# blue-yonder/tsfresh

Hardware: AMD Instinct MI355X
Metric: series/sec (ComprehensiveFCParameters, len=1024) (higher is better)
Workload: dtype f64; 1 GPU; 100000 series/GPU x len 1024 float32 i.i.d. N(0,1), ComprehensiveFCParameters (783 columns), inputs and outputs resident in HBM; n_series_per_gpu=100000, length=1024, n_cols=783, parallelism=ids1

## Files before the change

### __graft_entry__.py

```python
import os
import subprocess
import sys

ROOT = os.path.dirname(os.path.abspath(__file__))
if ROOT not in sys.path:
    sys.path.insert(0, ROOT)


def build():
    subprocess.check_call(["make", "-C", os.path.join(ROOT, "tsfresh_amd", "csrc"), "-j4"])
    subprocess.check_call(["make", "-C", os.path.join(ROOT, "tsfresh_amd", "csrc"), "lab"])
    sys.path.insert(0, os.path.join(ROOT, "tests"))
    import emul_lib
    emul_lib.load()
    import emul_pack_lib
    emul_pack_lib.load()
    import emul_pack_set_lib
    emul_pack_set_lib.load()
    import emul_pack_dense_lib
    emul_pack_dense_lib.load()
    import emul_roll_lib
    emul_roll_lib.load()
    import emul_mprofile_lib
    emul_mprofile_lib.load()
    import tsfresh_amd
    from tsfresh_amd import _native
    lib = _native.load()
    for sym in _native.EXPORTS:
        getattr(lib, sym)
    assert lib.tsfa_calc_count() > 70


def smoke():
    import numpy as np
    import pandas as pd

    sys.path.insert(0, os.path.join(ROOT, "tests"))
    from oracle.extract import oracle_matrix
    from parity import compare
    from tsfresh_amd import ComprehensiveFCParameters, _native, extract_features

    if _native.device_count() < 1:
        raise RuntimeError("smoke() needs a HIP device: tsfresh_amd has no CPU fallback")
    rng = np.random.default_rng(7)
    n_ids, length = 16, 256
    x = rng.standard_normal((n_ids, length), dtype=np.float32)
    df = pd.DataFrame({"id": np.repeat(np.arange(n_ids), length), "time": np.tile(np.arange(length), n_ids),
                       "value": x.reshape(-1)})
    params = ComprehensiveFCParameters()
    feats = extract_features(df, column_id="id", column_sort="time", default_fc_parameters=params, device=0)
    assert feats.shape == (n_ids, 783), feats.shape
    values = x.astype(np.float64).reshape(-1)
    offsets = np.arange(n_ids + 1, dtype=np.int64) * length
    names, want = oracle_matrix(values, offsets, params)
    got = feats[names].to_numpy()
    bad = compare(names, got, want, [values[offsets[i]:offsets[i + 1]] for i in range(n_ids)])
    if bad:
        raise AssertionError("%d mismatches vs oracle, e.g. %s" % (len(bad), bad[:5]))
    print("smoke ok: %d series x %d features match the oracle" % feats.shape)


if __name__ == "__main__":
    build()
    if len(sys.argv) > 1 and sys.argv[1] == "smoke":
        smoke()
```

### tsfresh_amd/csrc/fam_ar.h

```cpp
#ifndef TSFA_FAM_AR_H
#define TSFA_FAM_AR_H

#include "tsfa_common.h"

TSFA_DEV int adf_maxlag_for(int n) {
    int maxlag = (int)ceil(12.0 * pow((double)n / 100.0, 0.25));
    const int cap = n / 2 - 1 - 1;
    if (cap < maxlag) maxlag = cap;
    return maxlag;
}

TSFA_DEV int ar_tri(int i, int j) { return ((i * (i + 1)) >> 1) + j; }
TSFA_DEV int ar_tri_doubles(int P) { return (P * (P - 1)) / 2; }

TSFA_DEV void ar_sync(const Blk &b) {
#if TSFA_GPU && !defined(TSFA_LONG)
    if (b.nt <= 64) {
        asm volatile("s_waitcnt lgkmcnt(0)" ::: "memory");
        return;
    }
#endif
    (void)b;
    blk_sync();
}

TSFA_DEV bool chol_factor(double *G, int p) {
    for (int j = 0; j < p; ++j) {
        double d = G[ar_tri(j, j)];
        for (int k = 0; k < j; ++k) d -= G[ar_tri(j, k)] * G[ar_tri(j, k)];
        if (!(d > 0.0)) return false;
        d = sqrt(d);
        G[ar_tri(j, j)] = d;
        for (int i = j + 1; i < p; ++i) {
            double s = G[ar_tri(i, j)];
            for (int k = 0; k < j; ++k) s -= G[ar_tri(i, k)] * G[ar_tri(j, k)];
            G[ar_tri(i, j)] = s / d;
        }
    }
    return true;
}
TSFA_DEV void chol_solve(const double *L, int p, const double *rhs, double *x) {
    for (int i = 0; i < p; ++i) {
        double s = rhs[i];
        for (int k = 0; k < i; ++k) s -= L[ar_tri(i, k)] * x[k];
        x[i] = s * (1.0 / L[ar_tri(i, i)]);
    }
    for (int i = p - 1; i >= 0; --i) {
        double s = x[i];
        for (int k = i + 1; k < p; ++k) s -= L[ar_tri(k, i)] * x[k];
        x[i] = s * (1.0 / L[ar_tri(i, i)]);
    }
}

TSFA_DEV void blk_chol_solve(const Blk &b, const double *L, int p, const double *rhs, double *x) {
#if TSFA_GPU
    const int lane = b.tid & 63;
    const bool live = lane < p;
    double s = live ? rhs[lane] : 0.0;
    const double dg = live ? 1.0 / L[ar_tri(lane, lane)] : 1.0;
    for (int k = 0; k < p; ++k) {
        const double wk = readlane_f64(s, k) * readlane_f64(dg, k);
        if (lane == k) s = wk;
        else if (live && lane > k) s -= L[ar_tri(lane, k)] * wk;
    }
    for (int k = p - 1; k >= 0; --k) {
        const double xk = readlane_f64(s, k) * readlane_f64(dg, k);
        if (lane == k) s = xk;
        else if (live && lane < k) s -= L[ar_tri(k, lane)] * xk;
    }
    if (b.tid < p) x[b.tid] = s;
#else
    if (b.tid == 0) chol_solve(L, p, rhs, x);
#endif
}

#define TSFA_AR_PIVOT_TOL 1e-6
TSFA_DEV bool blk_chol_factor(const Blk &b, double *G, int p, double *diag0, double *dmin = nullptr) {
    for (int a = b.tid; a < p; a += b.nt) diag0[a] = G[ar_tri(a, a)];
    double dm = TSFA_INF;
    for (int j = 0; j < p; ++j) {
        ar_sync(b);
        const double d = G[ar_tri(j, j)];
        if (!(d > TSFA_AR_PIVOT_TOL * diag0[j])) return false;
        dm = fmin(dm, d);
        if (dmin) *dmin = dm;
        const double sd = sqrt(d);
        ar_sync(b);
        const double rsd = 1.0 / sd;
        for (int i = j + b.tid; i < p; i += b.nt) G[ar_tri(i, j)] = (i == j) ? sd : G[ar_tri(i, j)] * rsd;
        ar_sync(b);
        const int rsh = (b.nt >= 32) ? 5 : 0;
        for (int i = j + 1 + (b.tid & ((1 << rsh) - 1)); i < p; i += (1 << rsh)) {
            const double lij = G[ar_tri(i, j)];
            for (int k = j + 1 + (b.tid >> rsh); k <= i; k += (b.nt >> rsh))
                G[ar_tri(i, k)] = G[ar_tri(i, k)] - lij * G[ar_tri(k, j)];
        }
    }
    ar_sync(b);
    return true;
}
TSFA_DEV void blk_chol_forward(const Blk &b, const double *L, int p, double *w) {
#if TSFA_GPU
    if (p <= 64) {
        const int lane = b.tid & 63;
        const bool live = lane < p;
        double s = live ? w[lane] : 0.0;
        const double dg = live ? 1.0 / L[ar_tri(lane, lane)] : 1.0;
// ... 755 lines not shown
```

### tsfresh_amd/csrc/fam_sort.h

```cpp
#ifndef TSFA_FAM_SORT_H
#define TSFA_FAM_SORT_H

#include "tsfa_common.h"
#include "fam_langevin_dd.h"

template <class S>
TSFA_DEV double np_quantile_sorted(S s, int n, double q) {
    const double vi = (double)(n - 1) * q;
    int prev, next;
    double pf = floor(vi);
    if (vi >= (double)(n - 1)) {
        prev = next = n - 1;
        pf = -1.0;
    } else if (vi < 0.0) {
        prev = next = 0;
        pf = 0.0;
    } else {
        prev = (int)pf;
        next = prev + 1;
    }
    const double gamma = vi - pf;
    const double a = s(prev), c = s(next);
    const double diff = c - a;
    double r = a + diff * gamma;
// ... 154 lines not shown
#pragma unroll
    for (int j = 0; j < DD - 1; ++j) {
        int c = 0;
#pragma unroll
        for (int l = j + 1; l < DD; ++l) c += (r[l] < r[j]) ? 1 : 0;
        f /= (DD - j);
        code += c * f;
    }
    return code;
}
template <class AT>
TSFA_DEV int perm_code(const AT *a, int D, int fact) {
    switch (D) {
    case 2: return perm_code_fixed<2>(a, fact);
    case 3: return perm_code_fixed<3>(a, fact);
    case 4: return perm_code_fixed<4>(a, fact);
    case 5: return perm_code_fixed<5>(a, fact);
    case 6: return perm_code_fixed<6>(a, fact);
    case 7: return perm_code_fixed<7>(a, fact);
    default: break;
    }
    int code = 0, f = fact;
    for (int j = 0; j < D - 1; ++j) {
        int c = 0;
        for (int l = j + 1; l < D; ++l) c += ((double)a[l] < (double)a[j]) ? 1 : 0;
        f /= (D - j);
        code += c * f;
    }
    return code;
}

#define TSFA_FRIEDRICH_MAX_R 64
#define TSFA_FRIEDRICH_MAX_M 3

struct FrDefer {
    double *buf;
    int *count;
    int slot_doubles;
    long long sidx;
    int spec;
    int cap;
};

struct FxScale {
    int s1, s2;
};
TSFA_DEV FxScale fx_scale(double amax, int bits) {
    int e2 = 0;
    (void)frexp(amax, &e2);
    FxScale f;
    f.s1 = 60 - bits - e2;
    f.s2 = f.s1 + 59 - bits;
    return f;
}
TSFA_DEV void fx_split(double v, FxScale f, long long &hi, long long &lo) {
    const double h = rint(ldexp(v, f.s1));
    hi = (long long)h;
    lo = (long long)rint(ldexp(v - ldexp(h, -f.s1), f.s2));
}
TSFA_DEV double fx_value(long long hi, long long lo, FxScale f) {
    const long long hh = hi >> 26, hl = hi - hh * 67108864LL, lh = lo >> 26, ll = lo - lh * 67108864LL;
    const double a = ldexp((double)hh, 26 - f.s1), bq = ldexp((double)hl, -f.s1);
    const double c = ldexp((double)lh, 26 - f.s2), d = ldexp((double)ll, -f.s2);
    double s = c + d;
    double e = d - (s - c);
    double s2 = bq + s;
    double bb = s2 - bq;
    double e2 = (bq - (s2 - bb)) + (s - bb);
    double s3 = a + s2;
    bb = s3 - a;
    double e3 = (a - (s3 - bb)) + (s2 - bb);
    return s3 + (e3 + (e2 + e));
}

template <class XS, class S1>
TSFA_DEV bool friedrich_bin_means(const Blk &b, XS xs, int n, S1 srt1, int r, double *fw) {
    const int ns = n - 1;
    if (ns < 1 || r < 1) return false;
    double *edges = fw;
    double *sx = fw + (r + 1);
    double *sy = sx + r;
    double *cnt = sy + r;
    double *lows = cnt + r + 1;
    blk_sync();
    for (int j = b.tid; j <= r; j += b.nt) {
        const double q = np_linspace_at(0.0, 1.0, r + 1, j);
        edges[j] = pd_quantile_sorted(srt1, ns, q);
    }
    long long *isx = (long long *)(void *)sx, *isy = (long long *)(void *)sy, *icnt = (long long *)(void *)cnt,
              *isxl = (long long *)(void *)lows, *isyl = isxl + r;
    for (int j = b.tid; j < r; j += b.nt) { isx[j] = 0; isy[j] = 0; icnt[j] = 0; isxl[j] = 0; isyl[j] = 0; }
    blk_sync();
    double bad = 0.0;
    for (int j = b.tid; j < r; j += b.nt) bad += (edges[j] < edges[j + 1]) ? 0.0 : 1.0;
    bad = blk_sum(b, bad);
    if (bad > 0.0) return false;
    {
        double amax = fmax(fabs(srt1(0)), fabs(srt1(ns - 1)));
        amax = fmax(amax, fabs(xs[n - 1]));
        int bits = 1;
        while ((1 << bits) < n) ++bits;
        const FxScale fx = fx_scale(amax, bits), fy = fx_scale(2.0 * amax, bits);
        for (int i = b.tid; i < ns; i += b.nt) {
            const double x = xs[i];
            int lo = 0, hi = r + 1;
            while (lo < hi) {
                const int mid = (lo + hi) >> 1;
                if (edges[mid] < x) lo = mid + 1; else hi = mid;
            }
            int bin = lo - 1;
            if (x == edges[0]) bin = 0;
            if (bin < 0 || bin >= r) continue;
            const double dlt = xs[i + 1] - xs[i];
            long long xh, xl, yh, yl;
            fx_split(x, fx, xh, xl);
            fx_split(dlt, fy, yh, yl);
#if TSFA_GPU
            atomicAdd((unsigned long long *)&isx[bin], (unsigned long long)xh);
            atomicAdd((unsigned long long *)&isy[bin], (unsigned long long)yh);
            if (xl != 0) atomicAdd((unsigned long long *)&isxl[bin], (unsigned long long)xl);
            if (yl != 0) atomicAdd((unsigned long long *)&isyl[bin], (unsigned long long)yl);
            atomicAdd((unsigned long long *)&icnt[bin], 1ULL);
#else
            isx[bin] += xh; isy[bin] += yh; isxl[bin] += xl; isyl[bin] += yl; icnt[bin] += 1;
#endif
        }
        blk_sync();
        for (int j = b.tid; j < r; j += b.nt) {
            const double vx = fx_value(isx[j], isxl[j], fx), vy = fx_value(isy[j], isyl[j], fy);
            const double vc = (double)icnt[j];
            sx[j] = vx; sy[j] = vy; cnt[j] = vc;
        }
        blk_sync();
    }
    return true;
}

template <class XS, class S1>
TSFA_DEV void friedrich_coeffs(const Blk &b, XS xs, int n, S1 srt1, int m, int r,
                               double *fw, double *coef, const FrDefer &df) {
    for (int k = 0; k <= m; ++k) coef[k] = TSFA_NAN;
    const int ns = n - 1;
    if (ns < 1 || r < 1 || r > TSFA_FRIEDRICH_MAX_R || m < 1 || m > TSFA_FRIEDRICH_MAX_M) return;
    double *sx = fw + (r + 1);
    double *sy = sx + r;
    double *cnt = sy + r;
    double *flag = cnt + r;
    double *A = flag + 1;
    double *yv = A + r * (m + 1);
    double *cc = yv + r;
    double *tmp = cc + (m + 1);
    if (!friedrich_bin_means(b, xs, n, srt1, r, fw)) return;
    if (b.tid == 0) flag[0] = 0.0;
    blk_sync();
    const int rmax = (df.slot_doubles - TSFA_PF_HDR) / 2;
#if TSFA_GPU
    if (b.tid < 64) {
        const int lane = b.tid;
        const bool has = (lane < r) && (cnt[lane < r ? lane : 0] > 0.0);
        const unsigned long long mask = __ballot(has);
        const int k = __popcll(mask);
        const int cols = m + 1;
        const int row = has ? __popcll(mask & ((1ull << lane) - 1ull)) : 1000;
        const double xm = has ? sx[lane] / cnt[lane] : 0.0;
        const double ym = has ? sy[lane] / cnt[lane] : 0.0;
        bool defer = (k < cols);
        if (k >= cols) {
            double yrow = ym;
            double a[TSFA_FRIEDRICH_MAX_M + 1], scale[TSFA_FRIEDRICH_MAX_M + 1], R[TSFA_FRIEDRICH_MAX_M + 1][TSFA_FRIEDRICH_MAX_M + 1],
                qy[TSFA_FRIEDRICH_MAX_M + 1];
#pragma unroll
            for (int c = 0; c <= TSFA_FRIEDRICH_MAX_M; ++c) {
                a[c] = 0.0;
                scale[c] = 1.0;
                if (c < cols) {
                    double pw = 1.0;
                    for (int e = 0; e < m - c; ++e) pw *= xm;
                    pw = has ? pw : 0.0;
                    scale[c] = sqrt(wave_sum(pw * pw));
                    a[c] = pw / scale[c];
                    if (!has) a[c] = 0.0;
                }
            }
            double rmin = TSFA_INF, rbig = 0.0;
#pragma unroll
            for (int kk = 0; kk <= TSFA_FRIEDRICH_MAX_M; ++kk) {
                if (kk < cols) {
                    const bool below = has && (row >= kk);
                    const double nrm = sqrt(wave_sum(below ? a[kk] * a[kk] : 0.0));
                    const double akk = wave_sum((row == kk) ? a[kk] : 0.0);
                    if (nrm != 0.0) {
                        const double alpha = (akk > 0.0) ? -nrm : nrm;
                        const double v0 = akk - alpha;
                        const double vi = (row == kk) ? v0 : ((has && row > kk) ? a[kk] : 0.0);
                        const double vtv = wave_sum(vi * vi);
#pragma unroll
                        for (int j = 0; j <= TSFA_FRIEDRICH_MAX_M; ++j) {
                            if (j > kk && j < cols) {
                                const double d = 2.0 * wave_sum(vi * a[j]) / vtv;
                                a[j] -= d * vi;
                            }
                        }
                        const double d = 2.0 * wave_sum(vi * yrow) / vtv;
                        yrow -= d * vi;
                        R[kk][kk] = alpha;
                    } else {
                        R[kk][kk] = akk;
                    }
                    rmin = fmin(rmin, fabs(R[kk][kk]));
                    rbig = fmax(rbig, fabs(R[kk][kk]));
#pragma unroll
                    for (int j = 0; j <= TSFA_FRIEDRICH_MAX_M; ++j)
                        if (j > kk && j < cols) R[kk][j] = wave_sum((row == kk) ? a[j] : 0.0);
                    qy[kk] = wave_sum((row == kk) ? yrow : 0.0);
                }
            }
            double sol[TSFA_FRIEDRICH_MAX_M + 1];
#pragma unroll
            for (int kk = TSFA_FRIEDRICH_MAX_M; kk >= 0; --kk) {
                sol[kk] = 0.0;
                if (kk < cols) {
                    double sacc = qy[kk];
#pragma unroll
                    for (int j = 0; j <= TSFA_FRIEDRICH_MAX_M; ++j)
                        if (j > kk && j < cols) sacc -= R[kk][j] * sol[j];
                    sol[kk] = sacc / R[kk][kk];
                }
            }
            if (lane == 0) {
#pragma unroll
                for (int c = 0; c <= TSFA_FRIEDRICH_MAX_M; ++c)
                    if (c < cols) cc[c] = sol[c] / scale[c];
                flag[0] = 1.0;
            }
            defer = (rmin < TSFA_PF_FLAG * rbig);
        }
        if (defer && k >= 1) {
            if (df.buf != nullptr && r <= rmax) {
                int slot = 0;
                if (lane == 0) slot = atomicAdd(df.count, 1);
                slot = __shfl(slot, 0);
                if (slot < df.cap) {
                    double *rec = df.buf + (size_t)slot * (size_t)df.slot_doubles;
                    if (lane == 0) { rec[0] = (double)df.sidx; rec[1] = (double)df.spec; rec[2] = (double)k; }
                    if (has) { rec[TSFA_PF_HDR + row] = xm; rec[TSFA_PF_HDR + rmax + row] = ym; }
                }
            }
        }
    }
#else
    if (b.tid == 0) {
        int k = 0;
        double ysave[TSFA_FRIEDRICH_MAX_R];
        for (int j = 0; j < r; ++j) {
            if (cnt[j] > 0.0) {
                tmp[k] = sx[j] / cnt[j];
                yv[k] = sy[j] / cnt[j];
                ysave[k] = yv[k];
                ++k;
            }
        }
        const int cols = m + 1;
        double scale[TSFA_FRIEDRICH_MAX_M + 1];
        for (int c = 0; c < cols; ++c) {
            double ss = 0.0;
            for (int i = 0; i < k; ++i) {
                double pw = 1.0;
                for (int e = 0; e < m - c; ++e) pw *= tmp[i];
                A[i + c * k] = pw;
                ss += pw * pw;
            }
            scale[c] = sqrt(ss);
            for (int i = 0; i < k; ++i) A[i + c * k] /= scale[c];
        }
        bool defer = (k < cols);
        if (k >= cols) {
            double xsave[TSFA_FRIEDRICH_MAX_R];
            for (int i = 0; i < k; ++i) xsave[i] = tmp[i];
            small_lstsq(A, k, cols, yv, cc, tmp);
            for (int c = 0; c < cols; ++c) cc[c] = cc[c] / scale[c];
            flag[0] = 1.0;
            double rmin = TSFA_INF, rbig = 0.0;
            for (int c = 0; c < cols; ++c) {
                rmin = fmin(rmin, fabs(A[c + c * k]));
                rbig = fmax(rbig, fabs(A[c + c * k]));
            }
            defer = (rmin < TSFA_PF_FLAG * rbig);
            for (int i = 0; i < k; ++i) tmp[i] = xsave[i];
        }
        if (defer && k >= 1) {
            (void)rmax;
            double cf[TSFA_PF_MAXC];
            const double *tx = tmp;
            polyfit_svd_dd([=](int i) { return tx[i]; }, [=](int i) { return ysave[i]; }, k, m, cf);
            for (int c = 0; c < cols; ++c) cc[c] = cf[c];
            flag[0] = 1.0;
        }
    }
#endif
    blk_sync();
    if (flag[0] != 0.0)
        for (int c = 0; c <= m; ++c) coef[c] = cc[c];
    blk_sync();
}

#define TSFA_CQ_REFINE 9.5367431640625e-07
#ifdef TSFA_EMUL
static long long g_tsfa_cq_refined = 0;
#define TSFA_CQ_REFINE_NOTE() (++g_tsfa_cq_refined)
#else
#define TSFA_CQ_REFINE_NOTE() ((void)0)
#endif
struct CqRefined { double v, va; };
template <class XS>
TSFA_DEVN CqRefined cq_refine_corridor(const Blk &b, XS xs, int n, double l, double h, double mu1, double mu2, double c) {
    double e[4] = {0.0, 0.0, 0.0, 0.0};
    for (int i = b.tid; i < n - 1; i += b.nt) {
        const double x0 = xs[i], x1 = xs[i + 1];
        if (x0 >= l && x0 <= h && x1 >= l && x1 <= h) {
            const double d = x1 - x0;
            const double e1 = d - mu1, e2 = fabs(d) - mu2;
            e[0] += e1;
            e[1] += e1 * e1;
            e[2] += e2;
            e[3] += e2 * e2;
        }
    }
    blk_sum_multi<4>(b, e);
    CqRefined r;
    r.v = (e[1] - e[0] * e[0] / c) / c;
    r.va = (e[3] - e[2] * e[2] / c) / c;
    return r;
}
template <class XS, class SS>
TSFA_DEV void cq_fill_all(const Blk &b, XS xs, SS srt, int n, const TsfaCqPlan &plan, double *cq) {
    TSFA_TICKER(tkq, 0);
    for (int e0 = 0; e0 < 2 * plan.n; e0 += b.nt) {
        const int e = e0 + b.tid;
        double q = 0.0;
#if TSFA_GPU
        for (int c = 0; c < plan.n; ++c) {
            q = (e == c) ? plan.ql[c] : q;
            q = (e == plan.n + c) ? plan.qh[c] : q;
        }
#else
        if (e < 2 * plan.n) q = (e < plan.n) ? plan.ql[e] : plan.qh[e - plan.n];
#endif
        if (e < 2 * plan.n) {
            const double v = pd_quantile_sorted([=](int i) { return srt[i]; }, n, q);
            if (e < plan.n) cq[5 * e] = v; else cq[5 * (e - plan.n) + 1] = v;
        }
    }
    blk_sync();
    double s = (n > 1) ? (xs[n - 1] - xs[0]) / (double)(n - 1) : 0.0;
    if (!(fabs(s) <= 1.7976931348623157e308)) s = 0.0;
    const double sa = fabs(s);
    TSFA_TICK(tkq, b, 220);
    for (int k0 = 0; k0 < plan.n; k0 += 4) {
        const int ng = (plan.n - k0 < 4) ? (plan.n - k0) : 4;
        double lo[4], hi[4];
#pragma unroll
        for (int j = 0; j < 4; ++j) {
            const int k = (j < ng) ? (k0 + j) : k0;
            double l = cq[5 * k], h = cq[5 * k + 1];
#if TSFA_GPU
            l = readlane_f64(l, 0);
            h = readlane_f64(h, 0);
#endif
            lo[j] = (j < ng) ? l : TSFA_INF;
            hi[j] = (j < ng) ? h : -TSFA_INF;
        }
        double a[20];
#pragma unroll
        for (int k = 0; k < 20; ++k) a[k] = 0.0;
        for (int i = b.tid; i < n - 1; i += b.nt) {
            const double x0 = xs[i], x1 = xs[i + 1];
            const double d = x1 - x0;
            const double dd = d - s, ad = fabs(d) - sa;
            const double dd2 = dd * dd, ad2 = ad * ad;
#pragma unroll
            for (int j = 0; j < 4; ++j) {
                if (x0 >= lo[j] && x0 <= hi[j] && x1 >= lo[j] && x1 <= hi[j]) {
                    a[5 * j] += 1.0;
                    a[5 * j + 1] += dd;
                    a[5 * j + 2] += ad;
                    a[5 * j + 3] += dd2;
                    a[5 * j + 4] += ad2;
                }
            }
        }
        TSFA_TICK(tkq, b, 221);
        blk_sum_multi<20>(b, a);
        TSFA_TICK(tkq, b, 222);
        int refine = 0;
#pragma unroll
        for (int j = 0; j < 4; ++j) {
            const double c = a[5 * j], q1 = a[5 * j + 3] * c, q2 = a[5 * j + 4] * c;
            const bool many = c > 1.0;
            refine |= (many && q1 - a[5 * j + 1] * a[5 * j + 1] < TSFA_CQ_REFINE * q1) ? (1 << j) : 0;
            refine |= (many && q2 - a[5 * j + 2] * a[5 * j + 2] < TSFA_CQ_REFINE * q2) ? (16 << j) : 0;
        }
#if TSFA_GPU
        refine = __builtin_amdgcn_readfirstlane(refine);
#endif
        for (int j = 0; refine != 0 && j < ng; ++j) {
            if (((refine >> j) & 0x11) == 0) continue;
            TSFA_CQ_REFINE_NOTE();
            double l = lo[0], h = hi[0], c = a[0], t1 = a[1], t2 = a[2];
#pragma unroll
            for (int jj = 1; jj < 4; ++jj) {
                l = (jj == j) ? lo[jj] : l;
                h = (jj == j) ? hi[jj] : h;
                c = (jj == j) ? a[5 * jj] : c;
                t1 = (jj == j) ? a[5 * jj + 1] : t1;
                t2 = (jj == j) ? a[5 * jj + 2] : t2;
            }
            const CqRefined w = cq_refine_corridor(b, xs, n, l, h, s + t1 / c, sa + t2 / c, c);
            const double w1 = w.v, w2 = w.va;
#pragma unroll
            for (int jj = 0; jj < 4; ++jj) {
                a[5 * jj + 3] = (jj == j && ((refine >> jj) & 1)) ? w1 : a[5 * jj + 3];
                a[5 * jj + 4] = (jj == j && ((refine >> jj) & 16)) ? w2 : a[5 * jj + 4];
            }
        }
        blk_sync();
        if (b.tid == 0) {
#pragma unroll
            for (int j = 0; j < 4; ++j) {
                if (j < ng) {
                    double *o = cq + 5 * (k0 + j);
                    const double c = a[5 * j];
                    const bool any = c > 0.0;
                    const double m1 = any ? a[5 * j + 1] / c : 0.0, m2 = any ? a[5 * j + 2] / c : 0.0;
                    o[0] = c;
                    o[1] = any ? s + m1 : 0.0;
                    o[2] = any ? sa + m2 : 0.0;
                    double v1 = a[5 * j + 3] / c - m1 * m1, v2 = a[5 * j + 4] / c - m2 * m2;
                    v1 = ((refine >> j) & 1) ? a[5 * j + 3] : v1;
                    v2 = ((refine >> j) & 16) ? a[5 * j + 4] : v2;
                    o[3] = any ? ((v1 < 0.0) ? 0.0 : v1) : 0.0;
                    o[4] = any ? ((v2 < 0.0) ? 0.0 : v2) : 0.0;
                }
            }
        }
    }
    blk_sync();
}

enum { TSFA_SCTX_SYM = 0, TSFA_SCTX_NUNIQUE, TSFA_SCTX_MULTI_VALS, TSFA_SCTX_MULTI_PTS, TSFA_SCTX_SUM_VALS, TSFA_SCTX_SUM_PTS,
       TSFA_SORT_CTX = 8 };

template <class SS>
TSFA_DEV void sort_epilogue(const Blk &b, const TsfaSpec *specs, int first, int nspecs, int n, SS srt, const double *ctx,
                            const double *cq, double *out_row) {
    const double dn = (double)n;
    const double vmin = srt[0], vmax = srt[n - 1];
    for (int s = first + b.tid; s < nspecs; s += b.nt) {
        const TsfaSpec sp = specs[s];
        const double p0 = sp.p[0];
        double v = TSFA_NAN;
        switch (sp.calc) {
        case TSFA_C_MEDIAN: v = (n & 1) ? srt[(n - 1) / 2] : (0.0 + srt[n / 2 - 1] + srt[n / 2]) / 2.0; break;
        case TSFA_C_QUANTILE: v = np_quantile_sorted([=](int i) { return srt[i]; }, n, p0); break;
        case TSFA_C_SYMMETRY_LOOKING: v = (ctx[TSFA_SCTX_SYM] < p0 * (vmax - vmin)) ? 1.0 : 0.0; break;
        case TSFA_C_CHANGE_QUANTILES: {
            if (sp.p[1] != -2.0) { v = 0.0; break; }
            const double *o = cq + 5 * (((int)p0) & 127);
            const bool isabs = (sp.p[2] != 0.0);
            if (o[0] == 0.0) v = 0.0;
            else if ((int)sp.p[3] == TSFA_AGG_MEAN) v = isabs ? o[2] : o[1];
            else v = isabs ? o[4] : o[3];
        } break;
        case TSFA_C_HAS_DUPLICATE: v = (ctx[TSFA_SCTX_NUNIQUE] != dn) ? 1.0 : 0.0; break;
        case TSFA_C_RATIO_VALUE_NUMBER: v = ctx[TSFA_SCTX_NUNIQUE] / dn; break;
        case TSFA_C_PCT_REOCC_VALUES: v = ctx[TSFA_SCTX_MULTI_VALS] / ctx[TSFA_SCTX_NUNIQUE]; break;
        case TSFA_C_PCT_REOCC_DATAPOINTS: v = ctx[TSFA_SCTX_MULTI_PTS] / dn; break;
        case TSFA_C_SUM_REOCC_VALUES: v = ctx[TSFA_SCTX_SUM_VALS]; break;
        case TSFA_C_SUM_REOCC_DATA_POINTS: v = ctx[TSFA_SCTX_SUM_PTS]; break;
        default: break;
        }
        out_row[sp.col] = v;
    }
}

template <class ST>
TSFA_DEV void fam_sort_series(const Blk &b, const ST *xs_raw, int n, const TsfaSpec *specs, int nspecs,
                              double *out_row, ST *srt_raw, double *w, int *iw, const TsfaCqPlan &cqplan, double *cq,
                              TsfaSpec *stage, int n_loop = -1, double *ctx = nullptr, int w_doubles = 1280,
                              FrDefer df = FrDefer{nullptr, nullptr, TSFA_PF_HDR + 2 * TSFA_FRIEDRICH_MAX_R, 0, 0},
                              const unsigned short *perm_in = nullptr, const double *stats = nullptr, int pe_hint = 0) {
    const int hist_words = 2 * w_doubles;
    const int nloop = (n_loop >= 0 && ctx != nullptr) ? n_loop : nspecs;
    const XsView<ST> xs{xs_raw};
    const XsView<ST> srt{srt_raw};
    const int np2 = next_pow2(n);
    TSFA_TICKER(tk, 0);
    blk_sync();
    auto build_sorted_copy = [&]() {
        if (perm_in != nullptr && n >= 3) {
            for (int i = b.tid; i < np2; i += b.nt) srt_raw[i] = (i < n) ? xs_raw[perm_in[i]] : (ST)TSFA_INF;
            blk_sync();
        } else
#if TSFA_GPU
        if (!blk_sorted_copy_regs(b, xs_raw, n, srt_raw, np2))
#endif
        {
            for (int i = b.tid; i < np2; i += b.nt) srt_raw[i] = (i < n) ? xs_raw[i] : (ST)TSFA_INF;
            blk_bitonic_sort(b, srt_raw, np2);
        }
    };
    build_sorted_copy();
    TSFA_TICK(tk, b, 104);
    const double dn = (double)n;
    const double vmin = srt[0], vmax = srt[n - 1];

    bool have_sym = false, cq_valid = false, fr_valid = false;
    double sym_dist = 0.0, cq_ql = 0.0, cq_qh = 0.0, cq_cnt = 0.0, cq_mean = 0.0, cq_mean_abs = 0.0, cq_var = 0.0, cq_var_abs = 0.0;
    int fr_m = 0, fr_r = 0;
    double fr_coef[TSFA_FRIEDRICH_MAX_M + 1];

    double n_unique = 0.0, n_multi_vals = 0.0, n_multi_pts = 0.0, sum_multi_vals = 0.0, sum_multi_pts = 0.0;
    bool have_runs = false;

    for (int s = 0; s < nloop; ++s) {
        const TsfaSpec sp = spec_fetch(b, specs, nspecs, s, stage);
        const double p0 = sp.p[0], p1 = sp.p[1], p2 = sp.p[2], p3 = sp.p[3];
        double v = TSFA_NAN;
        switch (sp.calc) {
        case TSFA_C_MEDIAN:
            v = (n & 1) ? srt[(n - 1) / 2] : (0.0 + srt[n / 2 - 1] + srt[n / 2]) / 2.0;
            break;
        case TSFA_C_QUANTILE:
            v = np_quantile_sorted([=](int i) { return srt[i]; }, n, p0);
            break;
        case TSFA_C_SYMMETRY_LOOKING: {
            if (!have_sym) {
                const double mean = stats ? stats[TSFA_STATS_MEAN] : np_sum(b, n, [=](int i) { return xs[i]; }) / dn;
                const double med = (n & 1) ? srt[(n - 1) / 2] : (0.0 + srt[n / 2 - 1] + srt[n / 2]) / 2.0;
                sym_dist = fabs(mean - med);
                have_sym = true;
                if (nloop < nspecs && b.tid == 0) ctx[TSFA_SCTX_SYM] = sym_dist;
            }
            v = (sym_dist < p0 * (vmax - vmin)) ? 1.0 : 0.0;
        } break;
        case TSFA_C_MEAN_N_ABSOLUTE_MAX: {
            const int k = (int)p0;
            double r = TSFA_NAN;
            if (b.tid == 0 && n > k) {
                int lo = 0, hi = n - 1;
                double acc = 0.0;
                for (int t = 0; t < k; ++t) {
                    const double a = fabs(srt[lo]), c = fabs(srt[hi]);
                    if (a > c) { acc += a; ++lo; } else { acc += c; --hi; }
                }
                r = acc / (double)k;
            }
            v = blk_bcast0(b, r);
        } break;
        case TSFA_C_CHANGE_QUANTILES: {
            const double ql = p0, qh = p1;
            const bool isabs = (p2 != 0.0);
            const int agg = (int)p3;
            if (cqplan.n > 0 && p1 == -2.0) {
                if ((int)p0 >= 128) cq_fill_all(b, xs, srt, n, cqplan, cq);
                const double *o = cq + 5 * (((int)p0) & 127);
                if (o[0] == 0.0) v = 0.0;
                else if (agg == TSFA_AGG_MEAN) v = isabs ? o[2] : o[1];
                else v = isabs ? o[4] : o[3];
                break;
            }
            if (ql >= qh) { v = 0.0; break; }
            if (!(cq_valid && cq_ql == ql && cq_qh == qh)) {
                const double lo = pd_quantile_sorted([=](int i) { return srt[i]; }, n, ql);
                const double hi = pd_quantile_sorted([=](int i) { return srt[i]; }, n, qh);
                double c = 0.0, a = 0.0, aa = 0.0;
                for (int i = b.tid; i < n - 1; i += b.nt) {
                    const double x0 = xs[i], x1 = xs[i + 1];
                    if (x0 >= lo && x0 <= hi && x1 >= lo && x1 <= hi) {
                        const double d = x1 - x0;
                        c += 1.0;
                        a += d;
                        aa += fabs(d);
                    }
                }
                c = blk_sum(b, c);
                a = blk_sum(b, a);
                aa = blk_sum(b, aa);
                cq_cnt = c;
                cq_mean = (c > 0.0) ? a / c : 0.0;
                cq_mean_abs = (c > 0.0) ? aa / c : 0.0;
                double ss = 0.0, ssa = 0.0;
                if (c > 0.0) {
                    const double m1 = cq_mean, m2 = cq_mean_abs;
                    for (int i = b.tid; i < n - 1; i += b.nt) {
                        const double x0 = xs[i], x1 = xs[i + 1];
                        if (x0 >= lo && x0 <= hi && x1 >= lo && x1 <= hi) {
                            const double d = x1 - x0;
                            ss += (d - m1) * (d - m1);
                            ssa += (fabs(d) - m2) * (fabs(d) - m2);
                        }
                    }
                    ss = blk_sum(b, ss);
                    ssa = blk_sum(b, ssa);
                }
                cq_var = (c > 0.0) ? ss / c : 0.0;
                cq_var_abs = (c > 0.0) ? ssa / c : 0.0;
                cq_valid = true;
                cq_ql = ql;
                cq_qh = qh;
            }
            if (cq_cnt == 0.0) v = 0.0;
            else if (agg == TSFA_AGG_MEAN) v = isabs ? cq_mean_abs : cq_mean;
            else v = isabs ? cq_var_abs : cq_var;
        } break;
        case TSFA_C_HAS_DUPLICATE:
        case TSFA_C_RATIO_VALUE_NUMBER:
        case TSFA_C_PCT_REOCC_VALUES:
        case TSFA_C_PCT_REOCC_DATAPOINTS:
        case TSFA_C_SUM_REOCC_VALUES:
        case TSFA_C_SUM_REOCC_DATA_POINTS: {
            if (!have_runs) {
                double nu = 0.0, mv = 0.0, mp = 0.0, sv = 0.0, spn = 0.0;
                for (int i = b.tid; i < n; i += b.nt) {
                    const double x = srt[i];
                    const bool eq_prev = (i > 0) && (srt[i - 1] == x);
                    const bool eq_next = (i < n - 1) && (srt[i + 1] == x);
                    if (!eq_prev) {
                        nu += 1.0;
                        if (eq_next) { mv += 1.0; sv += x; }
                    }
                    if (eq_prev || eq_next) { mp += 1.0; spn += x; }
                }
                double r5[5] = {nu, mv, mp, sv, spn};
                blk_sum_multi<5>(b, r5);
                n_unique = r5[0]; n_multi_vals = r5[1]; n_multi_pts = r5[2]; sum_multi_vals = r5[3]; sum_multi_pts = r5[4];
                have_runs = true;
                if (nloop < nspecs && b.tid == 0) {
                    ctx[TSFA_SCTX_NUNIQUE] = n_unique; ctx[TSFA_SCTX_MULTI_VALS] = n_multi_vals;
                    ctx[TSFA_SCTX_MULTI_PTS] = n_multi_pts; ctx[TSFA_SCTX_SUM_VALS] = sum_multi_vals;
                    ctx[TSFA_SCTX_SUM_PTS] = sum_multi_pts;
                }
            }
            if (sp.calc == TSFA_C_HAS_DUPLICATE) v = (n_unique != dn) ? 1.0 : 0.0;
            else if (sp.calc == TSFA_C_RATIO_VALUE_NUMBER) v = n_unique / dn;
            else if (sp.calc == TSFA_C_PCT_REOCC_VALUES) v = n_multi_vals / n_unique;
            else if (sp.calc == TSFA_C_PCT_REOCC_DATAPOINTS) v = n_multi_pts / dn;
            else if (sp.calc == TSFA_C_SUM_REOCC_VALUES) v = sum_multi_vals;
            else v = sum_multi_pts;
        } break;
        case TSFA_C_PERMUTATION_ENTROPY: {
            const int tau = (int)p0, D = (int)p1;
            if (pe_hint != 0) { TSFA_TICK(tk, b, sp.calc); continue; }
            const int num = (n >= D) ? ((n - D) / tau + 1) : 0;
            if (num <= 0) { v = TSFA_NAN; break; }
            int fact = 1;
            for (int k = 2; k <= D; ++k) fact *= k;
            const bool wide = num > 65535;
            const int per_pass = wide ? hist_words : 2 * hist_words;
            if (fact > 16 * per_pass && sizeof(ST) >= sizeof(int)) {
                int *codes_s = (int *)(void *)srt_raw;
                const int cp2 = next_pow2(num);
                blk_sync();
                for (int t = b.tid; t < cp2; t += b.nt) codes_s[t] = (t < num) ? perm_code(xs_raw + t * tau, D, fact) : 0x7FFFFFFF;
                blk_bitonic_sort(b, codes_s, cp2);
                double es = 0.0;
                for (int t = b.tid; t < num; t += b.nt) {
                    const int c0 = codes_s[t];
                    if (t > 0 && codes_s[t - 1] == c0) continue;
                    int lo = t + 1, hi = num;
                    while (lo < hi) { const int mid = (lo + hi) >> 1; if (codes_s[mid] > c0) hi = mid; else lo = mid + 1; }
                    const double pr = (double)(lo - t) / (double)num;
                    es += pr * log(pr);
                }
                v = -blk_sum(b, es);
                blk_sync();
                build_sorted_copy();
                break;
            }
            const bool in_regs = (num <= 8 * b.nt);
            TSFA_TICKER(tp, 0);
            int codes[8];
            if (in_regs) {
#pragma unroll
                for (int u = 0; u < 8; ++u) {
                    const int t = b.tid + u * b.nt;
                    codes[u] = (t < num) ? perm_code(xs_raw + t * tau, D, fact) : -1;
                }
            }
            TSFA_TICK(tp, b, 236);
            const int LT = 64;
            double *ltab = b.np->leaf_sum;
            blk_sync();
            for (int c = b.tid; c < LT; c += b.nt) ltab[c] = (c > 0) ? log((double)c / (double)num) : 0.0;
            blk_sync();
            TSFA_TICK(tp, b, 237);
            double e = 0.0;
            for (int base = 0; base < fact; base += per_pass) {
                const int top = (fact - base < per_pass) ? (fact - base) : per_pass;
                blk_sync();
                for (int k = b.tid; k < (wide ? top : (top + 1) >> 1); k += b.nt) iw[k] = 0;
                blk_sync();
                if (in_regs) {
#pragma unroll
                    for (int u = 0; u < 8; ++u) {
                        const int c = codes[u] - base;
                        if (codes[u] >= 0 && c >= 0 && c < top) {
#if TSFA_GPU
                            if (wide) atomicAdd(&iw[c], 1); else atomicAdd(&iw[c >> 1], (c & 1) ? 0x10000 : 1);
#else
                            if (wide) iw[c] += 1; else iw[c >> 1] += (c & 1) ? 0x10000 : 1;
#endif
                        }
                    }
                } else {
                    for (int t = b.tid; t < num; t += b.nt) {
                        const int c = perm_code(xs_raw + t * tau, D, fact) - base;
                        if (c >= 0 && c < top) {
#if TSFA_GPU
                            if (wide) atomicAdd(&iw[c], 1); else atomicAdd(&iw[c >> 1], (c & 1) ? 0x10000 : 1);
#else
                            if (wide) iw[c] += 1; else iw[c >> 1] += (c & 1) ? 0x10000 : 1;
#endif
                        }
                    }
                }
                blk_sync();
                if (fact <= num) {
                    for (int k = b.tid; k < top; k += b.nt) {
                        const unsigned wv = (unsigned)iw[wide ? k : (k >> 1)];
                        const int c = wide ? (int)wv : ((k & 1) ? (int)(wv >> 16) : (int)(wv & 0xffffu));
                        if (c > 0) {
                            const double pr = (double)c / (double)num;
                            e += pr * ((c < LT) ? ltab[c] : log(pr));
                        }
                    }
                } else {
                    double acc = 0.0;
                    if (in_regs) {
#pragma unroll
                        for (int u = 0; u < 8; ++u) {
                            const int c = codes[u] - base;
                            if (codes[u] >= 0 && c >= 0 && c < top) {
                                const unsigned wv = (unsigned)iw[wide ? c : (c >> 1)];
                                const int cc = wide ? (int)wv : ((c & 1) ? (int)(wv >> 16) : (int)(wv & 0xffffu));
                                acc += (cc < LT) ? ltab[cc] : log((double)cc / (double)num);
                            }
                        }
                    } else {
                        for (int t = b.tid; t < num; t += b.nt) {
                            const int c = perm_code(xs_raw + t * tau, D, fact) - base;
                            if (c >= 0 && c < top) {
                                const unsigned wv = (unsigned)iw[wide ? c : (c >> 1)];
                                const int cc = wide ? (int)wv : ((c & 1) ? (int)(wv >> 16) : (int)(wv & 0xffffu));
                                acc += (cc < LT) ? ltab[cc] : log((double)cc / (double)num);
                            }
                        }
                    }
                    e += acc / (double)num;
                }
            }
            TSFA_TICK(tp, b, 238);
            v = -blk_sum(b, e);
            TSFA_TICK(tp, b, 239);
        } break;
        case TSFA_C_FRIEDRICH_COEFFICIENTS:
        case TSFA_C_MAX_LANGEVIN_FIXED_POINT: {
            int coeff, m, r;
            if (sp.calc == TSFA_C_FRIEDRICH_COEFFICIENTS) { coeff = (int)p0; m = (int)p1; r = (int)p2; }
            else { coeff = -1; m = (int)p0; r = (int)p1; }
            if (!(fr_valid && fr_m == m && fr_r == r)) {
                int pos = 0;
                {
                    const double xl = xs[n - 1];
                    int lo = 0, hi = n;
                    while (lo < hi) {
                        const int mid = (lo + hi) >> 1;
                        if (srt[mid] < xl) lo = mid + 1; else hi = mid;
                    }
                    pos = lo;
                }
                const XsView<ST> sr = srt;
                df.spec = s;
                friedrich_coeffs(b, xs, n, [=](int i) { return sr[i < pos ? i : i + 1]; }, m, r, w, fr_coef, df);
                fr_valid = true;
                fr_m = m;
                fr_r = r;
            }
            const double *coef = fr_coef;
            if (sp.calc == TSFA_C_FRIEDRICH_COEFFICIENTS) v = (coeff >= 0 && coeff <= m && m <= TSFA_FRIEDRICH_MAX_M) ? coef[coeff] : TSFA_NAN;
            else v = (m >= 1 && m <= TSFA_FRIEDRICH_MAX_M) ? max_real_root_deg3(coef, m + 1) : TSFA_NAN;
        } break;
        default: break;
        }
        if (b.tid == 0) out_row[sp.col] = v;
        TSFA_TICK(tk, b, sp.calc);
    }
    if (nloop < nspecs) {
        blk_sync();
        sort_epilogue(b, specs, nloop, nspecs, n, srt, ctx, cq, out_row);
    }
}

#endif
```

### tsfresh_amd/csrc/tsfa_api.cpp

```cpp
#include <hip/hip_runtime.h>

#include <stdio.h>
#include <stdlib.h>

#include <algorithm>
#include <string>
#include <vector>

#include "../../include/tsfresh_amd.h"
#include "tsfa_host_tables.h"
#include "tsfa_launch.h"
#include "fam_seq.h"
#include "tsfa_layout.h"

static thread_local std::string g_last_error;

static int fail(int code, const std::string &msg) {
    g_last_error = msg;
    return code;
}

int tsfa_fail(int code, const char *msg) { return fail(code, std::string(msg ? msg : "")); }
#define HIP_TRY(expr)                                                                                    \
    do {                                                                                                 \
        hipError_t e_ = (expr);                                                                          \
        if (e_ != hipSuccess) return fail(TSFA_ERR_HIP, std::string(#expr) + ": " + hipGetErrorString(e_)); \
    } while (0)

struct DevBuf {
    void *p = nullptr;
    size_t cap = 0;
    int ensure(size_t bytes) {
        if (bytes <= cap) return 0;
        size_t want = bytes + bytes / 8 + 4096;
        void *q = nullptr;
        if (hipMalloc(&q, want) != hipSuccess) {
            (void)hipGetLastError();
            if (p) { (void)hipFree(p); p = nullptr; cap = 0; }
            if (hipMalloc(&q, want) != hipSuccess) {
                (void)hipGetLastError();
                return -1;
            }
        }
        if (p) (void)hipFree(p);
        p = q;
        cap = want;
        return 0;
    }
    void release() {
        if (p) (void)hipFree(p);
        p = nullptr;
        cap = 0;
    }
};

#define TSFA_MAX_AUX 3
#define TSFA_MAX_CHUNKS 16
#define TSFA_DEFAULT_STREAMS 1

struct Timing {
    std::string name;
    hipEvent_t e0 = nullptr, e1 = nullptr;
    float ms = 0.f;
};

struct PlanOptions {
    bool length_classes = true;
    bool stats_share = true;
    bool perm_share = true;
    bool select = true;
    bool bluestein = true;
    bool cwt_mfma = false;
    bool force_long = false;
    int entropy_route = 0;
    int bluestein_min = 0;
    int gscratch_slots = 0;
    int host_chunks = 0;
    int nt[TSFA_N_FAMILIES] = {0};
    bool trace = false;
    bool row_form = true;
    int seq_rows = -1;
};

#if defined(TSFA_LAB)
#define TSFA_LAB_ONLY(x) (x)
#else
#define TSFA_LAB_ONLY(x) (0)
#endif

static int64_t g_relevance_batch = 0;
int64_t tsfa_relevance_batch_override() { return g_relevance_batch; }

struct tsfa_plan {
    int device = 0;
    PlanOptions opt;
    hipStream_t stream = nullptr;
    int n_cols = 0;
    std::vector<TsfaSpec> fam_specs[TSFA_N_FAMILIES];
    TsfaSpec *d_specs[TSFA_N_FAMILIES] = {nullptr};
    TsfaFamHints hints[TSFA_N_FAMILIES];
    TsfaCwtBank bank;
    double *d_W = nullptr;
    int *d_cols = nullptr, *d_coeff = nullptr;
    double *d_dectab = nullptr, *d_twc = nullptr, *d_tws = nullptr, *d_consts = nullptr;
    long long *d_stats = nullptr;
    DevBuf values, offsets, out, gscratch, times, deg_list, sel, long_scratch, pf_buf, perm_buf, stats_buf, dd_scratch, gen_scratch, seq_rows;
    std::vector<TsfaSpec> gen_specs;
    TsfaSpec *d_gen_specs = nullptr;
    TsfaGenPlan gen_plan;
    double *d_pool = nullptr;
    int *d_deg_count = nullptr;
    int *d_cursor = nullptr;
    hipStream_t s_in = nullptr, s_out = nullptr;
    hipEvent_t ev_in[TSFA_MAX_CHUNKS] = {nullptr}, ev_k[TSFA_MAX_CHUNKS] = {nullptr};
    std::vector<int64_t> h_rel;
    bool needs_times = false;
    bool sort_only_order_stats = false;
    bool stream_ok = false;
    int n_streams = 1;
    hipStream_t aux[TSFA_MAX_AUX] = {nullptr};
    hipEvent_t ev_fork = nullptr, ev_join[TSFA_MAX_AUX] = {nullptr};
    bool profiling = false;
    std::vector<Timing> timings;
    std::vector<tsfa_launch_info> launches;
    long long hint_min_len = 0, hint_max_len = 0;
    bool fill_all = false;
    int *d_fill_cols = nullptr;
    int n_fill_cols = 0;
    int debug_skip_fam = -1;
    hipStream_t side = nullptr;
    hipEvent_t ev_side_fork = nullptr, ev_side_join = nullptr;
    unsigned side_mask = 0;
    double fill_value = __builtin_nan("");
};

static const char *fam_names[TSFA_N_FAMILIES] = {"k_basic", "k_sort", "k_spectral", "k_ar", "k_entropy", "k_cwtpeaks", "k_seq", "k_trend", "k_mprofile"};

template <class T>
static int upload(const std::vector<T> &h, T **d) {
    *d = nullptr;
    if (h.empty()) return 0;
    if (hipMalloc((void **)d, h.size() * sizeof(T)) != hipSuccess) return -1;
    if (hipMemcpy(*d, h.data(), h.size() * sizeof(T), hipMemcpyHostToDevice) != hipSuccess) return -1;
    return 0;
}

static int record(tsfa_plan *plan, hipStream_t st, size_t slot, const char *name, bool begin) {
    if (!plan->profiling) return 0;
    if (plan->timings.size() <= slot) plan->timings.resize(slot + 1);
    Timing &t = plan->timings[slot];
    if (!t.e0) {
        if (hipEventCreate(&t.e0) != hipSuccess || hipEventCreate(&t.e1) != hipSuccess) return -1;
// ... 157 lines not shown
    for (int f = 0; ok && f < TSFA_N_FAMILIES; ++f) ok = upload(plan->fam_specs[f], &plan->d_specs[f]) == 0;
    if (ok) ok = upload(plan->gen_specs, &plan->d_gen_specs) == 0;
    if (ok && n_data > 0) ok = upload(std::vector<double>(data, data + n_data), &plan->d_pool) == 0;
    if (ok && !cwt_coef.empty()) {
        ok = upload(plan->bank.W, &plan->d_W) == 0 && upload(plan->bank.cols, &plan->d_cols) == 0 &&
             upload(plan->bank.coeff_idx, &plan->d_coeff) == 0;
    }
    if (ok) {
        std::vector<double> dt, twc, tws;
        tsfa_build_dectab(dt);
        tsfa_build_twiddles(twc, tws);
        ok = upload(dt, &plan->d_dectab) == 0 && upload(twc, &plan->d_twc) == 0 && upload(tws, &plan->d_tws) == 0;
        std::vector<double> consts;
        tsfa_build_consts(consts);
        ok = ok && upload(consts, &plan->d_consts) == 0;
    }
    if (ok) ok = hipMalloc((void **)&plan->d_stats, TSFA_LEN_STATS * sizeof(long long)) == hipSuccess;
    if (ok) ok = hipMalloc((void **)&plan->d_deg_count, 2 * sizeof(int)) == hipSuccess;
    if (ok) ok = hipMalloc((void **)&plan->d_cursor, TSFA_N_LEN_CLASSES * sizeof(int)) == hipSuccess;
    if (ok) ok = hipStreamCreateWithFlags(&plan->s_in, hipStreamNonBlocking) == hipSuccess &&
                 hipStreamCreateWithFlags(&plan->s_out, hipStreamNonBlocking) == hipSuccess;
    for (int i = 0; ok && i < TSFA_MAX_CHUNKS; ++i)
        ok = hipEventCreateWithFlags(&plan->ev_in[i], hipEventDisableTiming) == hipSuccess &&
             hipEventCreateWithFlags(&plan->ev_k[i], hipEventDisableTiming) == hipSuccess;
    {
        const char *e = getenv("TSFA_STREAMS");
        plan->n_streams = e ? std::min(std::max(atoi(e), 1), TSFA_MAX_AUX + 1) : TSFA_DEFAULT_STREAMS;
        for (int i = 0; ok && i + 1 < plan->n_streams; ++i)
            ok = hipStreamCreateWithFlags(&plan->aux[i], hipStreamNonBlocking) == hipSuccess &&
                 hipEventCreateWithFlags(&plan->ev_join[i], hipEventDisableTiming) == hipSuccess;
        if (ok && plan->n_streams > 1) ok = hipEventCreateWithFlags(&plan->ev_fork, hipEventDisableTiming) == hipSuccess;
    }
    if (const char *e = getenv("TSFA_PAIR")) {
        static const char *nm[TSFA_N_FAMILIES] = {"basic", "sort", "spectral", "ar", "entropy", "cwt", "seq", "trend", "mprofile"};
        for (int f = 0; f < TSFA_N_FAMILIES; ++f)
            if (f != TSFA_FAM_BASIC && f != TSFA_FAM_SORT && f != TSFA_FAM_ENTROPY && strstr(e, nm[f])) plan->side_mask |= 1u << f;
        if (plan->side_mask) {
            int least = 0, greatest = 0;
            (void)hipDeviceGetStreamPriorityRange(&least, &greatest);
            ok = ok && hipStreamCreateWithPriority(&plan->side, hipStreamNonBlocking, least) == hipSuccess &&
                 hipEventCreateWithFlags(&plan->ev_side_fork, hipEventDisableTiming) == hipSuccess &&
                 hipEventCreateWithFlags(&plan->ev_side_join, hipEventDisableTiming) == hipSuccess;
        }
    }
    if (const char *e = getenv("TSFA_HOST_CHUNKS")) plan->opt.host_chunks = std::max(atoi(e), 0);
    if (!ok) {
        tsfa_plan_destroy(plan);
        return fail(TSFA_ERR_HIP, "device allocation/upload failed while creating the plan");
    }
    *out_plan = plan;
    return TSFA_OK;
}

int32_t tsfa_plan_n_cols(const tsfa_plan *plan) { return plan ? plan->n_cols : -1; }

int tsfa_plan_set_length_hint(tsfa_plan *plan, int64_t min_len, int64_t max_len) {
    if (!plan) return fail(TSFA_ERR_INVALID, "null plan");
    if (max_len == 0 && min_len == 0) { plan->hint_min_len = plan->hint_max_len = 0; return TSFA_OK; }
    if (min_len < 1 || max_len < min_len || max_len > 2147483647LL / 64) return fail(TSFA_ERR_INVALID, "length hint must satisfy 1 <= min <= max <= 33554431");
    plan->hint_min_len = min_len;
    plan->hint_max_len = max_len;
    return TSFA_OK;
}

int tsfa_plan_set_option(tsfa_plan *plan, const char *name, double value) {
    if (!name) return fail(TSFA_ERR_INVALID, "option name is NULL");
    const std::string n(name);
    const bool on = value != 0.0;
    if (!plan) {
        if (n == "relevance_batch") { g_relevance_batch = value > 0.0 ? (int64_t)value : 0; return TSFA_OK; }
        return fail(TSFA_ERR_INVALID, "unknown library option '" + n + "'");
    }
    PlanOptions &o = plan->opt;
    if (n == "length_classes") o.length_classes = on;
    else if (n == "stats_share") o.stats_share = on;
    else if (n == "perm_share") o.perm_share = on;
    else if (n == "select") o.select = on;
    else if (n == "bluestein") o.bluestein = on;
    else if (n == "cwt_mfma") o.cwt_mfma = on;
    else if (n == "force_long") o.force_long = on;
    else if (n == "row_form") o.row_form = on;
    else if (n == "seq_rows") o.seq_rows = (value < 0.0) ? -1 : (on ? 1 : 0);
    else if (n == "entropy_route") { if (value != 0.0 && value != 1.0 && value != 2.0) return fail(TSFA_ERR_INVALID, "entropy_route: 0, 1 or 2"); o.entropy_route = (int)value; }
    else if (n == "bluestein_min") o.bluestein_min = value > 0.0 ? (int)std::min(value, 32767.0) : 0;
    else if (n == "gscratch_slots") o.gscratch_slots = value > 0.0 ? (int)std::min(value, 2147483647.0) : 0;
    else if (n == "host_chunks") o.host_chunks = value > 0.0 ? (int)std::min(value, (double)TSFA_MAX_CHUNKS) : 0;
    else if (n == "fused_minimal") { if (!on) plan->stream_ok = false; }
    else if (n == "perm_fused") { if (!on) plan->hints[TSFA_FAM_SORT].d = 0; }
    else if (n == "fill") { plan->fill_value = value; plan->fill_all = true; }
    else if (n == "fill_off") { plan->fill_all = false; }
#if defined(TSFA_LAB)
    else if (n == "skip_family") plan->debug_skip_fam = (int)value;
    else if (n == "trace") o.trace = on;
    else if (n.rfind("nt_", 0) == 0 && n.size() == 4 && n[3] >= '0' && n[3] < '0' + TSFA_N_FAMILIES) o.nt[n[3] - '0'] = (int)value;
#endif
    else return fail(TSFA_ERR_INVALID, "unknown plan option '" + n + "'");
    return TSFA_OK;
}

int tsfa_plan_set_profiling(tsfa_plan *plan, int32_t enable) {
    if (!plan) return fail(TSFA_ERR_INVALID, "plan is NULL");
    plan->profiling = enable != 0;
    return TSFA_OK;
}

int32_t tsfa_plan_last_timings(const tsfa_plan *plan, const char **names, float *ms, int32_t cap) {
    if (!plan) return 0;
    int32_t n = 0;
    for (const auto &t : plan->timings) {
        if (n >= cap) break;
        if (names) names[n] = t.name.c_str();
        if (ms) ms[n] = t.ms;
        ++n;
    }
    return n;
}

int32_t tsfa_plan_last_launches(const tsfa_plan *plan, tsfa_launch_info *out, int32_t cap) {
    if (!plan) return 0;
    const int32_t n = (int32_t)plan->launches.size();
    for (int32_t i = 0; out && i < n && i < cap; ++i) out[i] = plan->launches[(size_t)i];
    return n;
}

int tsfa_extract(tsfa_plan *plan, const void *values, int32_t dtype, const int64_t *offsets, int64_t n_series,
                 double *out, int64_t ld_out, int32_t space, void *stream) {
    return tsfa_extract_timed(plan, values, dtype, nullptr, offsets, n_series, out, ld_out, space, stream);
}

int tsfa_extract_timed(tsfa_plan *plan, const void *values, int32_t dtype, const double *times, const int64_t *offsets,
                       int64_t n_series, double *out, int64_t ld_out, int32_t space, void *stream) {
    return tsfa_extract_windows(plan, values, dtype, times, offsets, offsets ? offsets + 1 : nullptr, n_series, out,
                                ld_out, space, stream);
}

struct BatchShape {
    long long max_len = 0, min_len = 0, max_np2 = 0;
    int n_groups = 1;
    int g_maxn[TSFA_N_LEN_CLASSES] = {0};
    long long g_np2[TSFA_N_LEN_CLASSES] = {0};
    int64_t g_count[TSFA_N_LEN_CLASSES] = {0};
    bool g_has_short[TSFA_N_LEN_CLASSES] = {false};
    TsfaClassMap map;
};

static void shape_from_stats(const long long *st, int64_t n_series, BatchShape &sh, bool length_classes) {
    sh.max_len = st[0];
    sh.min_len = st[1];
    sh.max_np2 = st[2];
    memset(&sh.map, 0, sizeof sh.map);
    sh.n_groups = 1;
    sh.g_maxn[0] = (int)st[0];
    sh.g_np2[0] = st[2];
    sh.g_count[0] = n_series;
    sh.g_has_short[0] = st[1] <= TSFA_ROW_MAXN;
    if (!length_classes || n_series < 2048 || st[0] <= 2 * st[1] || st[0] <= 128) return;
    const int64_t min_group = 512;
    int ng = 0;
    int64_t pend_count = 0;
    long long pend_np2 = 0;
    int first_of_group = 0;
    for (int c = 0; c < TSFA_N_LEN_CLASSES; ++c) {
        const int64_t cnt = st[3 + c];
        pend_count += cnt;
        pend_np2 = std::max(pend_np2, st[3 + 2 * TSFA_N_LEN_CLASSES + c]);
        bool last = true;
// ... 61 lines not shown

static int run_batch(tsfa_plan *plan, const void *d_values, int dtype, const double *d_times, const int64_t *d_starts,
                     const int64_t *d_ends, int64_t n_series, double *d_out, int64_t ld, const BatchShape &sh,
                     const int *d_sel, hipStream_t st, bool with_overlap) {
    if ((plan->fill_all || plan->n_fill_cols > 0) &&
        tsfa_launch_fill_nan(d_out, n_series, plan->n_cols, ld, st, plan->fill_value, plan->fill_all ? nullptr : plan->d_fill_cols,
                             plan->n_fill_cols))
        return fail(TSFA_ERR_HIP, "fill launch failed");

    static const int order_long_first[TSFA_N_FAMILIES] = {TSFA_FAM_ENTROPY, TSFA_FAM_AR, TSFA_FAM_SORT, TSFA_FAM_CWT, TSFA_FAM_BASIC,
                                                          TSFA_FAM_SEQ, TSFA_FAM_SPECTRAL, TSFA_FAM_TREND, TSFA_FAM_MPROFILE};
    static const int order_basic_first[TSFA_N_FAMILIES] = {TSFA_FAM_BASIC, TSFA_FAM_ENTROPY, TSFA_FAM_AR, TSFA_FAM_SORT, TSFA_FAM_CWT,
                                                           TSFA_FAM_SEQ, TSFA_FAM_SPECTRAL, TSFA_FAM_TREND, TSFA_FAM_MPROFILE};
    const bool overlap = with_overlap && plan->n_streams > 1 && !plan->profiling;
    const bool share_stats = plan->stats_buf.p != nullptr && !overlap && !plan->stream_ok && plan->opt.stats_share;
    const int *order = share_stats ? order_basic_first : order_long_first;
    bool stats_valid[TSFA_N_LEN_CLASSES + 1];
    for (int g = 0; g <= TSFA_N_LEN_CLASSES; ++g) stats_valid[g] = false;
    if (overlap) {
        HIP_TRY(hipEventRecord(plan->ev_fork, st));
        for (int i = 0; i + 1 < plan->n_streams; ++i) HIP_TRY(hipStreamWaitEvent(plan->aux[i], plan->ev_fork, 0));
    }
    bool pair = plan->side != nullptr && plan->side_mask != 0 && !overlap && !plan->profiling && with_overlap;
    for (int g = 0; g < sh.n_groups; ++g) pair = pair && sh.g_maxn[g] <= 4096;
    bool side_forked = false, side_used = false;
    size_t slot = 0;
    int dealt = 0;
    bool perm_valid[TSFA_N_LEN_CLASSES + 1];
    for (int g = 0; g <= TSFA_N_LEN_CLASSES; ++g) perm_valid[g] = false;
    const bool perm_share = plan->perm_buf.p != nullptr && !overlap && plan->opt.perm_share;
    bool stream_done[TSFA_N_LEN_CLASSES + 1];
    for (int g = 0; g <= TSFA_N_LEN_CLASSES; ++g) stream_done[g] = false;
    for (int fi = 0; fi < TSFA_N_FAMILIES; ++fi) {
        const int f = order[fi];
        if (plan->fam_specs[f].empty()) continue;
        if (TSFA_LAB_ONLY(plan->debug_skip_fam == f)) continue;
        if (f == TSFA_FAM_BASIC && plan->stream_ok) {
            bool all = true;
            for (int g = 0; g < sh.n_groups; ++g) all = all && stream_done[g];
            if (all) continue;
        }
        hipStream_t fst = st;
        if (overlap) {
            const int k = dealt++ % plan->n_streams;
            if (k > 0) fst = plan->aux[k - 1];
        }
        if (pair && fi > 0 && ((plan->side_mask >> f) & 1u)) {
            if (!side_forked) {
                HIP_TRY(hipEventRecord(plan->ev_side_fork, st));
                HIP_TRY(hipStreamWaitEvent(plan->side, plan->ev_side_fork, 0));
                side_forked = true;
            }
            fst = plan->side;
            side_used = true;
        }
        const char *slot_name = (plan->stream_ok && (f == TSFA_FAM_SORT || (f == TSFA_FAM_BASIC && plan->fam_specs[TSFA_FAM_SORT].empty())))
                                    ? "k_stream" : fam_names[f];
        if (record(plan, fst, slot, slot_name, true)) return fail(TSFA_ERR_HIP, "event record failed");
        std::vector<TsfaLaunch> perm_launches;
        for (int g = sh.n_groups - 1; g >= 0; --g) {
            const int maxn = sh.g_maxn[g];
            const long long max_np2 = sh.g_np2[g];
            TsfaLaunch a;
            memset(&a, 0, sizeof a);
            a.fam = f;
            a.dtype = dtype;
            a.values = d_values;
            a.starts = d_starts;
            a.ends = d_ends;
            a.n_series = sh.g_count[g];
            a.sel = (sh.n_groups > 1) ? d_sel + sh.map.base[g] : nullptr;
            a.specs = plan->d_specs[f];
            a.nspecs = (int)plan->fam_specs[f].size();
            a.out = d_out;
            a.ld = ld;
            a.maxn = maxn;
            a.nt = (maxn <= 2048) ? 64 : 256;
            if (maxn > 2048) {
                static const int nt_8k[TSFA_N_FAMILIES] = {512, 512, 512, 512, 256, 1024, 256, 256, 256};
                static const int nt_4k[TSFA_N_FAMILIES] = {256, 256, 256, 256, 256, 512, 256, 256, 256};
                a.nt = (maxn > 4096) ? nt_8k[f] : nt_4k[f];
            }
            if (maxn <= 2048) {
                static const int pref[TSFA_N_FAMILIES] = {64, 128, 128, 64, 256, 256, 128, 64, 256};
                const int cap = std::max(64, ((maxn / 4 + 63) / 64) * 64);
                a.nt = std::min(pref[f], cap);
            }
            if (TSFA_LAB_ONLY(plan->opt.nt[f] >= 64)) a.nt = plan->opt.nt[f];
            a.stream = fst;
            a.dectab = plan->d_dectab;
            a.times = d_times;
            a.twc = plan->d_twc;
            a.consts = plan->d_consts;
            a.tws = plan->d_tws;
            a.hint_a = plan->hints[f].a;
            a.hint_b = plan->hints[f].b;
            a.hint_c = plan->hints[f].c;
            a.hint_d = plan->hints[f].d;
            a.hint_e = plan->hints[f].e;
            a.alt = plan->hints[f].alt;
            a.cq = plan->hints[f].cq;
            if (f == TSFA_FAM_SPECTRAL && maxn > 2048 && !TSFA_LAB_ONLY(plan->opt.nt[f] >= 64)) a.nt = 512;
            int aux = 0;
            if (f == TSFA_FAM_TREND) aux = a.alt.small_w;
            if (f == TSFA_FAM_MPROFILE) aux = (dtype == TSFA_F32) ? 4 : 8;
            if (f == TSFA_FAM_SPECTRAL) {
                a.dft_n = (int)std::min<long long>(max_np2, 256);
                aux = a.dft_n;
                int bl_odd = TSFA_BLUESTEIN_MIN, bl_even = TSFA_BLUESTEIN_MIN_EVEN;
                if (plan->opt.bluestein_min > 0) bl_odd = bl_even = std::min(std::max(plan->opt.bluestein_min, 17), 32767);
                a.bluestein_min = TSFA_BLUESTEIN_PACK(bl_odd, bl_even);
                if (max_np2 >= std::min(bl_odd, bl_even) && max_np2 <= 32768 && plan->opt.bluestein) {
                    long long M = 1;
                    while (M < 2 * max_np2 - 1) M <<= 1;
                    const size_t slot_bytes = (size_t)(4 * M) * sizeof(double);
                    int64_t slots = std::min<int64_t>(a.n_series, std::max<int64_t>((int64_t)((1ull << 30) / slot_bytes), 2048));
                    if (plan->opt.gscratch_slots > 0) slots = std::min<int64_t>(slots, plan->opt.gscratch_slots);
                    const size_t bytes = (size_t)slots * slot_bytes;
                    if (plan->gscratch.ensure(bytes) == 0) {
                        a.gscratch = (double *)plan->gscratch.p;
                        a.gscratch_n = (int)(4 * M);
                        a.gscratch_slots = slots;
                    }
                }
            } else if (f == TSFA_FAM_CWT) {
                a.cwt_rowv = tsfa_family_lds_bytes(f, maxn, a.nt, 1) <= 96 * 1024 ? 1 : 0;
                aux = a.cwt_rowv;
                if (plan->opt.cwt_mfma) a.cwt_rowv |= 2;
            } else if (f == TSFA_FAM_AR) {
                int P = 8, Pdd = 8;
                for (const auto &s : plan->fam_specs[f]) {
                    if (s.calc == TSFA_C_AUGMENTED_DICKEY_FULLER) {
                        int ml = (int)ceil(12.0 * pow((double)maxn / 100.0, 0.25));
                        if (maxn / 2 - 2 < ml) ml = maxn / 2 - 2;
                        P = std::max(P, ml + 3);
                    } else if (s.calc == TSFA_C_AR_COEFFICIENT) {
                        const int k = std::min((int)s.p[1], std::max(1, (maxn - 2) / 2));
                        if ((int)s.p[1] <= TSFA_AR_TABLE_K) P = std::max(P, (int)s.p[1] + 2);
                        Pdd = std::max(Pdd, k + 2);
                        a.ar_has_coef = 1;
                    }
                }
                Pdd = std::max(Pdd, P);
                a.ar_P = P;
                a.ar_P_dd = Pdd;
                aux = P;
                {
                    ArDdLds D;
                    if (D.carve(nullptr, Pdd) > TSFA_LDS_LIMIT - 2048) {
                        const size_t slot_bytes = (size_t)ArDdLds::scratch_doubles(Pdd) * sizeof(double);
                        const int slots = (int)std::min<int64_t>(a.n_series, std::min<int64_t>(256, std::max<int64_t>(8, (int64_t)(((size_t)2 << 30) / slot_bytes))));
                        if (plan->dd_scratch.ensure((size_t)slots * slot_bytes))
                            return fail(TSFA_ERR_HIP, "hipMalloc failed for the second AR pass");
                        a.dd_scratch = (double *)plan->dd_scratch.p;
                        a.dd_slots = slots;
                    }
                }
                a.deg_list = (long long *)plan->deg_list.p;
                a.deg_count = plan->d_deg_count;
                HIP_TRY(hipMemsetAsync(plan->d_deg_count, 0, sizeof(int), fst));
            } else if (f == TSFA_FAM_SORT && plan->hints[f].b > 0) {
                a.pf_slot = tsfa_pf_slot_doubles(plan->hints[f].b);
                a.pf_buf = (double *)plan->pf_buf.p;
                a.pf_count = plan->d_deg_count + 1;
                a.pf_cap = (int)std::min<long long>((long long)n_series * std::max(1, plan->hints[f].e), 2147483647LL);
                HIP_TRY(hipMemsetAsync(a.pf_count, 0, sizeof(int), fst));
            } else if (f == TSFA_FAM_ENTROPY) {
                const int waves = std::min(4, std::max(1, (maxn - 1 + 63) / 64));
                a.nt = std::max(a.nt, 64 * waves);
// ... 52 lines not shown
                    for (int s0 = 0; s0 < a.nspecs; s0 += group_g) {
                        lz_build_group(plan->fam_specs[f].data() + s0, std::min(group_g, a.nspecs - s0), maxn, &g, 1);
                        lds_g = std::max(lds_g, tsfa_seq_lds_bytes(g));
                        stride_g = std::max(stride_g, (size_t)g.stride);
                    }
                    auto resident = [&](size_t lds) {
                        if (lds > TSFA_LDS_LIMIT) return (size_t)0;
                        return std::min<size_t>((size_t)(163840 / std::max<size_t>(lds, 1)), (size_t)(32 * 64 / a.nt));
                    };
                    const bool more = resident(lds_g) > resident(seq_lds);
                    if (lds_g <= TSFA_LDS_LIMIT && (plan->opt.seq_rows == 1 || more) &&
                        (size_t)a.n_series * stride_g <= ((size_t)2 << 30) &&
                        plan->seq_rows.ensure((size_t)a.n_series * stride_g) == 0) {
                        seq_grows = 1;
                        seq_group = group_g;
                        seq_lds = lds_g;
                        a.seq_rows = (unsigned char *)plan->seq_rows.p;
                    }
                }
            }
            size_t lds = (f == TSFA_FAM_SEQ) ? seq_lds
                         : (f == TSFA_FAM_ENTROPY) ? tsfa_entropy_lds_bytes(maxn, a.ent_cnt)
                                                   : tsfa_family_lds_bytes(f, maxn, a.nt, aux);
            const bool use_long = lds > TSFA_LDS_LIMIT || plan->opt.force_long || (f == TSFA_FAM_ENTROPY && a.ent_cnt == 4);
            if (TSFA_LAB_ONLY(f == TSFA_FAM_SPECTRAL && plan->opt.trace))
                fprintf(stderr, "[tsfa] spectral group %d: n_series %lld maxn %d max_np2 %lld lds %zu long %d chirp-z %d slots %lld nt %d\n", g,
                        (long long)a.n_series, maxn, max_np2, lds, (int)use_long, (int)(a.gscratch != nullptr), (long long)a.gscratch_slots, a.nt);
            if (use_long) {
                if (!(f == TSFA_FAM_ENTROPY && a.ent_cnt == 4)) a.nt = 256;
                if (a.gscratch != nullptr && a.gscratch_slots < std::min<int64_t>(a.n_series, 2048)) a.gscratch = nullptr;
                if (f == TSFA_FAM_ENTROPY && a.ent_cnt != 4) { a.ent_cnt = 0; a.ent_fast = 0; lds = tsfa_entropy_lds_bytes(maxn, 5); }
                if (f == TSFA_FAM_CWT) { a.cwt_rowv &= 2; lds = tsfa_family_lds_bytes(f, maxn, a.nt, 0); }
                if (f == TSFA_FAM_SEQ) {
                    seq_group = std::min(a.nspecs, TSFA_LZ_MAX_GROUP);
                    seq_grows = 0;
                    lds = 0;
                    for (int s0 = 0; s0 < a.nspecs; s0 += seq_group) {
                        lz_build_group(plan->fam_specs[f].data() + s0, std::min(seq_group, a.nspecs - s0), maxn, &a.seq);
                        lds = std::max(lds, tsfa_seq_lds_bytes(a.seq));
                    }
                } else if (f != TSFA_FAM_ENTROPY && f != TSFA_FAM_CWT) {
                    lds = tsfa_family_lds_bytes(f, maxn, a.nt, aux);
                }
                const size_t slot_bytes = (lds + 255) & ~(size_t)255;
                const int64_t n_slots = std::max<int64_t>(1, std::min<int64_t>(std::min<int64_t>(a.n_series, 512),
                                                                               (int64_t)((4ull << 30) / slot_bytes)));
                if (plan->long_scratch.ensure((size_t)n_slots * slot_bytes))
                    return fail(TSFA_ERR_HIP, "hipMalloc failed for the long-series scratch");
                a.long_scratch = (unsigned char *)plan->long_scratch.p;
                a.long_bytes = (size_t)n_slots * slot_bytes;
            }
            if (share_stats && g <= TSFA_N_LEN_CLASSES) {
                if (f == TSFA_FAM_BASIC && !(plan->hints[f].c == 0 && a.nt <= 256)) {
                    a.stats_out = (double *)plan->stats_buf.p;
                    stats_valid[g] = true;
                } else if ((f == TSFA_FAM_ENTROPY || f == TSFA_FAM_AR || f == TSFA_FAM_SEQ || f == TSFA_FAM_SORT) && stats_valid[g]) {
                    a.stats_in = (const double *)plan->stats_buf.p;
                }
            }
            if (perm_share && !use_long && g <= TSFA_N_LEN_CLASSES) {
                if (f == TSFA_FAM_ENTROPY && a.ent_cnt == 2 && maxn <= TSFA_ENTB_MAXN) {
                    a.perm_buf = (unsigned short *)plan->perm_buf.p;
                    a.perm_stride = TSFA_ENTB_MAXN;
                    perm_valid[g] = true;
                } else if (f == TSFA_FAM_SORT && perm_valid[g]) {
                    a.perm_buf = (unsigned short *)plan->perm_buf.p;
                    a.perm_stride = TSFA_ENTB_MAXN;
                }
            }
            if (f == TSFA_FAM_SORT) {
                a.hint_d = 0;
                if (plan->hints[f].d != 0) {
                    const int pnt = (maxn <= 2048) ? std::min(256, std::max(64, ((maxn / 4 + 63) / 64) * 64))
                                                   : std::min(1024, ((maxn / 8 + 63) / 64) * 64);
                    if (maxn <= 65535 && tsfa_perm_lds_bytes(maxn, pnt, dtype == TSFA_F32 ? 4 : 8) <= TSFA_LDS_LIMIT) {
                        a.hint_d = plan->hints[f].d;
                        TsfaLaunch pa = a;
                        pa.nt = pnt;
                        pa.long_scratch = nullptr;
                        perm_launches.push_back(pa);
                    }
                }
            }
            if (!(plan->stream_ok && (f == TSFA_FAM_SORT || f == TSFA_FAM_BASIC) && maxn <= 2048 && g <= TSFA_N_LEN_CLASSES && stream_done[g])) {
                tsfa_launch_info li;
                li.family = f;
                li.length_class = g;
                li.max_len = maxn;
                li.threads = a.nt;
                li.n_series = a.n_series;
                li.lds_bytes = (int64_t)lds;
                li.long_build = use_long ? 1 : 0;
                li.variant = (f == TSFA_FAM_ENTROPY) ? a.ent_cnt
                             : (f == TSFA_FAM_CWT) ? a.cwt_rowv
                             : (f == TSFA_FAM_SEQ) ? (seq_group | (seq_grows << 8))
                             : (f == TSFA_FAM_SPECTRAL) ? (a.gscratch != nullptr ? 1 : 0)
                             : (f == TSFA_FAM_SORT) ? (a.hint_d != 0 ? 1 : 0)
                             : (f == TSFA_FAM_AR) ? (a.dd_scratch != nullptr ? 1 : 0) : 0;
                plan->launches.push_back(li);
            }
            int rc = 0;
            if (plan->stream_ok && (f == TSFA_FAM_SORT || f == TSFA_FAM_BASIC) && maxn <= 2048 && g <= TSFA_N_LEN_CLASSES) {
                if (stream_done[g]) continue;
                TsfaLaunch sa = a;
                sa.specs = plan->d_specs[TSFA_FAM_SORT];
                sa.nspecs = (int)plan->fam_specs[TSFA_FAM_SORT].size();
                sa.bspecs = plan->d_specs[TSFA_FAM_BASIC];
                sa.nbspecs = (int)plan->fam_specs[TSFA_FAM_BASIC].size();
                rc = tsfa_launch_stream(sa);
                stream_done[g] = true;
            } else
            if (f == TSFA_FAM_SORT && plan->sort_only_order_stats && maxn <= 2048 && !use_long &&
                plan->opt.select) {
                rc = tsfa_launch_order_stats(a);
            } else if (f == TSFA_FAM_SEQ) {
                for (int s0 = 0; rc == 0 && s0 < a.nspecs; s0 += seq_group) {
                    lz_build_group(plan->fam_specs[f].data() + s0, std::min(seq_group, a.nspecs - s0), maxn, &a.seq, seq_grows);
                    if (!use_long && tsfa_seq_lds_bytes(a.seq) > TSFA_LDS_LIMIT)
                        return fail(TSFA_ERR_TOO_LONG, "k_seq: a series of " + std::to_string(maxn) + " samples does not fit LDS");
                    rc = use_long ? tsfa_launch_family_long(a) : tsfa_launch_family(a);
                }
            } else {
                bool rows_any = false, rows_all = false;
                const bool lite = (f == TSFA_FAM_BASIC && plan->hints[f].c == 0 && a.nt <= 256);
                if ((f == TSFA_FAM_BASIC || f == TSFA_FAM_TREND) && plan->opt.row_form && !lite && g <= TSFA_N_LEN_CLASSES) {
                    rows_any = sh.g_has_short[g];
                    rows_all = maxn <= TSFA_ROW_MAXN;
                }
                if (rows_any) {
                    a.skip_le = TSFA_ROW_MAXN;
                    rc = tsfa_launch_rows(a);
                }
                if (rc == 0 && !rows_all) rc = use_long ? tsfa_launch_family_long(a) : tsfa_launch_family(a);
            }
            if (rc == 0 && f == TSFA_FAM_AR) rc = tsfa_launch_ar_degenerate(a);
            if (rc == 0 && f == TSFA_FAM_SORT && a.pf_buf) rc = tsfa_launch_langevin_dd(a);
            if (rc) return fail(TSFA_ERR_HIP, std::string(fam_names[f]) + " launch failed: " +
                                                  (rc == -2 ? "no scratch slot" : hipGetErrorString((hipError_t)rc)));
        }
        if (record(plan, fst, slot, slot_name, false)) return fail(TSFA_ERR_HIP, "event record failed");
        ++slot;
        if (!perm_launches.empty()) {
            if (record(plan, fst, slot, "k_perm", true)) return fail(TSFA_ERR_HIP, "event record failed");
            for (const auto &pa : perm_launches) {
                const int rc = tsfa_launch_perm(pa);
                if (rc) return fail(TSFA_ERR_HIP, std::string("k_perm launch failed: ") + hipGetErrorString((hipError_t)rc));
            }
            if (record(plan, fst, slot, "k_perm", false)) return fail(TSFA_ERR_HIP, "event record failed");
            ++slot;
        }
    }
    if (overlap) {
        for (int i = 0; i + 1 < plan->n_streams; ++i) {
            HIP_TRY(hipEventRecord(plan->ev_join[i], plan->aux[i]));
            HIP_TRY(hipStreamWaitEvent(st, plan->ev_join[i], 0));
        }
    }
    if (side_used) {
        HIP_TRY(hipEventRecord(plan->ev_side_join, plan->side));
        HIP_TRY(hipStreamWaitEvent(st, plan->ev_side_join, 0));
    }
    if (plan->bank.C > 0) {
        TsfaCwtLaunch c;
        memset(&c, 0, sizeof c);
        c.dtype = dtype;
        c.values = d_values;
        c.starts = d_starts;
        c.ends = d_ends;
        c.n_series = n_series;
        c.W = plan->d_W;
        c.S4 = plan->bank.S4;
        c.C = plan->bank.C;
        c.cols = plan->d_cols;
        c.coeff_idx = plan->d_coeff;
        c.out = d_out;
        c.ld = ld;
        c.stream = st;
        if (record(plan, st, slot, "k_cwt_gemm", true)) return fail(TSFA_ERR_HIP, "event record failed");
        const int rc = tsfa_launch_cwt(c);
        if (rc) return fail(TSFA_ERR_HIP, "k_cwt_gemm launch failed");
// ... 237 lines not shown
```

### tsfresh_amd/csrc/tsfa_common.h

```cpp
#ifndef TSFA_COMMON_H
#define TSFA_COMMON_H

#include <math.h>
#include <stdint.h>

#include "tsfa_specs.h"

#if defined(__HIPCC__)
#include <hip/hip_runtime.h>
#define TSFA_GPU 1
#define TSFA_DEV __device__ __forceinline__
#define TSFA_DEVN __device__ __noinline__
#define TSFA_MEM __device__ __forceinline__
#else
#define TSFA_GPU 0
#define TSFA_DEV static inline
#define TSFA_DEVN static
#define TSFA_MEM inline
#endif
#if defined(__HIP_DEVICE_COMPILE__)
#define TSFA_ASSUME_LDS(p) __builtin_assume(__builtin_amdgcn_is_shared((const void *)(p)))
#else
#define TSFA_ASSUME_LDS(p) ((void)0)
#endif
// ... 7 lines not shown
struct NpScratch {
    double leaf_sum[TSFA_NP_MAXLEAF];
    double vst[32];
    int leaf_off[TSFA_NP_MAXLEAF];
    int leaf_len[TSFA_NP_MAXLEAF];
    int st_o[32], st_l[32], st_v[32];
    int nleaf;
    int pad;
    double result;
};

template <typename ST>
struct XsView {
    typedef ST elem;
    const ST *p;
    TSFA_MEM double operator[](int i) const { return (double)p[i]; }
};

struct Blk {
    int tid;
    int nt;
    double *red;
    NpScratch *np;
};

#define TSFA_ROW_MAXN 256
#define TSFA_ROW_LANES 16
struct BlkRow : Blk {};
template <class BT> struct BlkLanes { static constexpr int n = 64; };
template <> struct BlkLanes<BlkRow> { static constexpr int n = TSFA_ROW_LANES; };
template <class BT> struct BlkIsRow { static constexpr bool v = false; };
template <> struct BlkIsRow<BlkRow> { static constexpr bool v = true; };
TSFA_DEV Blk blk_rebind(const Blk &b, int tid) { return Blk{tid, b.nt, b.red, b.np}; }
TSFA_DEV BlkRow blk_rebind(const BlkRow &b, int tid) { BlkRow r; r.tid = tid; r.nt = b.nt; r.red = b.red; r.np = b.np; return r; }

#if TSFA_GPU && defined(TSFA_TICKS)
static __device__ unsigned long long tsfa_ticks[256];
static __shared__ unsigned long long tsfa_ticks_lds[256];
struct Ticker {
    unsigned long long t;
    int base;
    __device__ __forceinline__ explicit Ticker(int base_) : t(__builtin_readcyclecounter()), base(base_) {}
    __device__ __forceinline__ void mark(int tid, int id) {
        const unsigned long long now = __builtin_readcyclecounter();
        if (tid == 0) tsfa_ticks_lds[base + id] += now - t;
        t = __builtin_readcyclecounter();
    }
};
#define TSFA_TICKER(name, base) Ticker name(base)
#define TSFA_TICK(name, b, id) name.mark((b).tid, id)
#define TSFA_TICKS_BEGIN()                                                                  \
    do {                                                                                    \
        for (int i_ = threadIdx.x; i_ < 256; i_ += blockDim.x) tsfa_ticks_lds[i_] = 0ull;   \
        __syncthreads();                                                                    \
    } while (0)
#define TSFA_TICKS_END()                                                                    \
    do {                                                                                    \
        __syncthreads();                                                                    \
        for (int i_ = threadIdx.x; i_ < 256; i_ += blockDim.x)                              \
            if (tsfa_ticks_lds[i_]) atomicAdd(&tsfa_ticks[i_], tsfa_ticks_lds[i_]);         \
    } while (0)
#else
#define TSFA_TICKER(name, base)
#define TSFA_TICK(name, b, id)
#define TSFA_TICKS_BEGIN()
#define TSFA_TICKS_END()
#endif

TSFA_DEV void blk_sync() {
#if TSFA_GPU
#if defined(TSFA_LONG)
    asm volatile("s_waitcnt vmcnt(0) lgkmcnt(0)" ::: "memory");
    __syncthreads();
#else
    asm volatile("s_waitcnt lgkmcnt(0)\n\ts_barrier" ::: "memory");
#endif
#endif
}
TSFA_DEV void blk_sync_all() {
#if TSFA_GPU
    asm volatile("s_waitcnt vmcnt(0) lgkmcnt(0)" ::: "memory");
    __syncthreads();
#endif
}

#if TSFA_GPU
template <int CTRL>
TSFA_DEV double dpp_mov_f64(double v) {
    union { double d; int i[2]; } a, r;
    a.d = v;
    r.i[0] = __builtin_amdgcn_update_dpp(a.i[0], a.i[0], CTRL, 0xf, 0xf, false);
    r.i[1] = __builtin_amdgcn_update_dpp(a.i[1], a.i[1], CTRL, 0xf, 0xf, false);
    return r.d;
}
TSFA_DEV double readlane_f64(double v, int lane) {
    union { double d; int i[2]; } a, r;
    a.d = v;
    r.i[0] = __builtin_amdgcn_readlane(a.i[0], lane);
    r.i[1] = __builtin_amdgcn_readlane(a.i[1], lane);
    return r.d;
}
#define TSFA_DPP_QUAD_XOR1 0xB1
#define TSFA_DPP_QUAD_XOR2 0x4E
#define TSFA_DPP_ROW_HALF_MIRROR 0x141
#define TSFA_DPP_ROW_MIRROR 0x140
TSFA_DEV double wave_sum(double v) {
    v += dpp_mov_f64<TSFA_DPP_QUAD_XOR1>(v);
    v += dpp_mov_f64<TSFA_DPP_QUAD_XOR2>(v);
    v += dpp_mov_f64<TSFA_DPP_ROW_HALF_MIRROR>(v);
    v += dpp_mov_f64<TSFA_DPP_ROW_MIRROR>(v);
    return (readlane_f64(v, 0) + readlane_f64(v, 16)) + (readlane_f64(v, 32) + readlane_f64(v, 48));
}
TSFA_DEV double wave_min(double v) {
    v = fmin(v, dpp_mov_f64<TSFA_DPP_QUAD_XOR1>(v));
    v = fmin(v, dpp_mov_f64<TSFA_DPP_QUAD_XOR2>(v));
    v = fmin(v, dpp_mov_f64<TSFA_DPP_ROW_HALF_MIRROR>(v));
    v = fmin(v, dpp_mov_f64<TSFA_DPP_ROW_MIRROR>(v));
    return fmin(fmin(readlane_f64(v, 0), readlane_f64(v, 16)), fmin(readlane_f64(v, 32), readlane_f64(v, 48)));
}
TSFA_DEV double wave_max(double v) {
    v = fmax(v, dpp_mov_f64<TSFA_DPP_QUAD_XOR1>(v));
    v = fmax(v, dpp_mov_f64<TSFA_DPP_QUAD_XOR2>(v));
    v = fmax(v, dpp_mov_f64<TSFA_DPP_ROW_HALF_MIRROR>(v));
    v = fmax(v, dpp_mov_f64<TSFA_DPP_ROW_MIRROR>(v));
    return fmax(fmax(readlane_f64(v, 0), readlane_f64(v, 16)), fmax(readlane_f64(v, 32), readlane_f64(v, 48)));
}
#endif

TSFA_DEV double blk_sum(const Blk &b, double v) {
#if TSFA_GPU
    v = wave_sum(v);
    if (b.nt > 64) {
        const int nw = b.nt >> 6;
        blk_sync();
        if ((b.tid & 63) == 0) b.red[b.tid >> 6] = v;
        blk_sync();
        v = b.red[0];
        for (int w = 1; w < nw; ++w) v += b.red[w];
    }
#endif
    return v;
}
#define TSFA_SPEC_BATCH 16
TSFA_DEV TsfaSpec spec_fetch(const Blk &b, const TsfaSpec *specs, int nspecs, int s, TsfaSpec *stage) {
#if TSFA_GPU && defined(TSFA_SPEC_LDS)
    if ((s % TSFA_SPEC_BATCH) == 0) {
        blk_sync();
        const int cnt = (nspecs - s < TSFA_SPEC_BATCH) ? (nspecs - s) : TSFA_SPEC_BATCH;
        const double *src = (const double *)(const void *)(specs + s);
        double *dst = (double *)(void *)stage;
        for (int i = b.tid; i < cnt * (int)(sizeof(TsfaSpec) / sizeof(double)); i += b.nt) dst[i] = src[i];
        blk_sync();
    }
    const TsfaSpec *e = stage + (s % TSFA_SPEC_BATCH);
    TsfaSpec r;
    r.calc = __builtin_amdgcn_readfirstlane(e->calc);
    r.col = __builtin_amdgcn_readfirstlane(e->col);
#pragma unroll
    for (int k = 0; k < 4; ++k) r.p[k] = readlane_f64(e->p[k], 0);
    return r;
#else
    (void)b; (void)nspecs; (void)stage;
    return specs[s];
#endif
}

// ... 474 lines not shown
                    s->st_l[sp] = n2;
                    s->st_v[sp] = 0;
                    ++sp;
                } else {
                    --sp;
                    const double r = s->vst[--vp];
                    const double lft = s->vst[--vp];
                    s->vst[vp++] = lft + r;
                }
            }
            const double chunk = s->vst[0];
            s->result = chunk;
        }
        blk_sync();
        total = (c0 == 0) ? s->result : (total + s->result);
    }
    blk_sync();
    return total;
}

#if TSFA_GPU
template <class F>
TSFA_DEV double np_row_leaves(int lane, int o, int l, F f) {
    const int k = lane & 7;
    double r = 0.0;
    if (l >= 8) {
        const int lim = l - (l % 8);
        r = f(o + k);
        for (int i = 8; i < lim; i += 8) r += f(o + i + k);
    }
    r += dpp_mov_f64<TSFA_DPP_QUAD_XOR1>(r);
    r += dpp_mov_f64<TSFA_DPP_QUAD_XOR2>(r);
    r += dpp_mov_f64<TSFA_DPP_ROW_HALF_MIRROR>(r);
    if (k == 0) {
        if (l < 8) {
            r = 0.0;
            for (int i = 0; i < l; ++i) r += f(o + i);
        } else {
            for (int i = l - (l % 8); i < l; ++i) r += f(o + i);
        }
    }
    return r;
}
template <class F>
TSFA_DEV double np_sum(const BlkRow &b, int n, F f) {
    if (n <= 0) return 0.0;
    const int lane = b.tid;
    int o1 = 0, l1 = 0, o2 = 0, l2 = 0, l0 = n, nleaf = 1;
    if (n > 128) {
        int h = n / 2;
        h -= h % 8;
        l0 = h;
        o1 = h;
        l1 = n - h;
        nleaf = 2;
        if (l1 > 128) {
            int h2 = l1 / 2;
            h2 -= h2 % 8;
            o2 = o1 + h2;
            l2 = l1 - h2;
            l1 = h2;
            nleaf = 3;
        }
    }
    const bool second = lane >= 8;
    const double a = np_row_leaves(lane, second ? o1 : 0, second ? l1 : l0, f);
    const double s0 = row_bcast_f64(a, 0), s1 = row_bcast_f64(a, 8);
    double s2 = 0.0;
    if (nleaf == 3) s2 = row_bcast_f64(np_row_leaves(lane, o2, second ? 0 : l2, f), 0);
    return (nleaf == 1) ? s0 : (nleaf == 2) ? (s0 + s1) : (s0 + (s1 + s2));
}
#endif

TSFA_DEV int next_pow2(int n) {
    int p = 1;
    while (p < n) p <<= 1;
    return p;
}

template <typename K>
TSFA_DEV void blk_bitonic_sort(const Blk &b, K *a, int npow2) {
    for (int k = 2; k <= npow2; k <<= 1) {
        for (int j = k >> 1; j > 0; j >>= 1) {
            blk_sync();
            for (int t = b.tid; t < (npow2 >> 1); t += b.nt) {
                const int i = ((t & ~(j - 1)) << 1) | (t & (j - 1));
                const int l = i | j;
                const bool up = ((i & k) == 0);
                const K x = a[i], y = a[l];
                if ((x > y) == up) {
                    a[i] = y;
                    a[l] = x;
                }
            }
        }
    }
    blk_sync();
}

template <class IDX>
TSFA_DEV void blk_argsort_idx(const Blk &b, const double *key, int n, IDX *perm, int np2) {
    const IDX none = (IDX)~(IDX)0;
    blk_sync();
    for (int i = b.tid; i < np2; i += b.nt) perm[i] = (i < n) ? (IDX)i : none;
    for (int k = 2; k <= np2; k <<= 1) {
        for (int j = k >> 1; j > 0; j >>= 1) {
            blk_sync();
            for (int t = b.tid; t < (np2 >> 1); t += b.nt) {
                const int i = ((t & ~(j - 1)) << 1) | (t & (j - 1));
                const int l = i | j;
                const bool up = ((i & k) == 0);
                const IDX a = perm[i], c = perm[l];
                const double ka = (a == none) ? TSFA_INF : key[a], kc = (c == none) ? TSFA_INF : key[c];
                const bool gt = (ka > kc) || (ka == kc && a > c);
                if (gt == up) {
                    perm[i] = c;
                    perm[l] = a;
                }
            }
        }
    }
    blk_sync();
}
TSFA_DEV void blk_argsort_u16(const Blk &b, const double *key, int n, unsigned short *perm, int np2) {
    blk_argsort_idx<unsigned short>(b, key, n, perm, np2);
}

#if TSFA_GPU
TSFA_DEV bool sort_pair_gt(double ka, int ia, double kb, int ib) { return (ka > kb) || (ka == kb && ia > ib); }

template <int E, int J>
TSFA_DEV void sort_stage_regs(double (&key)[E], int (&idx)[E], int g0, int k) {
#pragma unroll
    for (int e = 0; e < E; ++e) {
        if ((e & J) != 0) continue;
        const int f = e | J;
        const bool up = (((g0 + e) & k) == 0);
        const bool gt = sort_pair_gt(key[e], idx[e], key[f], idx[f]);
        if (gt == up) {
            const double tk = key[e]; key[e] = key[f]; key[f] = tk;
            const int ti = idx[e]; idx[e] = idx[f]; idx[f] = ti;
        }
    }
}

template <int LX>
TSFA_DEV int lane_xor_i32(int v) {
    if (LX == 1) return __builtin_amdgcn_update_dpp(v, v, TSFA_DPP_QUAD_XOR1, 0xf, 0xf, false);
    if (LX == 2) return __builtin_amdgcn_update_dpp(v, v, TSFA_DPP_QUAD_XOR2, 0xf, 0xf, false);
    if (LX == 16) {
        const auto r = __builtin_amdgcn_permlane16_swap(v, v, false, false);
        return ((threadIdx.x >> 4) & 1) ? (int)r[0] : (int)r[1];
    }
    if (LX == 32) {
        const auto r = __builtin_amdgcn_permlane32_swap(v, v, false, false);
        return ((threadIdx.x >> 5) & 1) ? (int)r[0] : (int)r[1];
    }
    if (LX == 8) return __builtin_amdgcn_update_dpp(v, v, 0x128 , 0xf, 0xf, false);
    if (LX == 4) {
        const int t = __builtin_amdgcn_update_dpp(v, v, 0x104 , 0xf, 0x5, false);
        return __builtin_amdgcn_update_dpp(t, v, 0x114 , 0xf, 0xa, false);
    }
    return __shfl_xor(v, LX);
}
template <int LX>
TSFA_DEV double lane_xor_f64(double v) {
    union { double d; int i[2]; } a, r;
    a.d = v;
    r.i[0] = lane_xor_i32<LX>(a.i[0]);
    r.i[1] = lane_xor_i32<LX>(a.i[1]);
    return r.d;
}

template <int E, int LX>
TSFA_DEV void sort_stage_lanes(double (&key)[E], int (&idx)[E], int g0, int k, int j) {
    const bool lower = ((g0 & j) == 0);
#pragma unroll
    for (int e = 0; e < E; ++e) {
        const double pk = lane_xor_f64<LX>(key[e]);
        const int pi = lane_xor_i32<LX>(idx[e]);
// ... 96 lines not shown
                switch (j / E) {
                case 1: sortp_stage_lanes<E, 1>(pk, g0, k, j); break;
                case 2: sortp_stage_lanes<E, 2>(pk, g0, k, j); break;
                case 4: sortp_stage_lanes<E, 4>(pk, g0, k, j); break;
                case 8: sortp_stage_lanes<E, 8>(pk, g0, k, j); break;
                case 16: sortp_stage_lanes<E, 16>(pk, g0, k, j); break;
                default: sortp_stage_lanes<E, 32>(pk, g0, k, j); break;
                }
            } else {
                blk_sync();
#pragma unroll
                for (int e = 0; e < E; ++e) xchg_idx[g0 + e] = (unsigned short)(pk[e] & 0xFFFFull);
                blk_sync();
                const bool lower = ((g0 & j) == 0);
#pragma unroll
                for (int e = 0; e < E; ++e) {
                    const int pi = xchg_idx[(g0 + e) ^ j];
                    const unsigned long long o = sort_pack_f32(keyof(pi), pi);
                    const bool up = (((g0 + e) & k) == 0);
                    const bool take = ((pk[e] > o) == (lower == up));
                    pk[e] = take ? o : pk[e];
                }
            }
        }
    }
}

TSFA_DEV float sort_min(float a, float b) { return __builtin_fminf(a, b); }
TSFA_DEV float sort_max(float a, float b) { return __builtin_fmaxf(a, b); }
TSFA_DEV double sort_min(double a, double b) { return __builtin_fmin(a, b); }
TSFA_DEV double sort_max(double a, double b) { return __builtin_fmax(a, b); }
template <int LX>
TSFA_DEV float lane_xor_key(float v) { return __int_as_float(lane_xor_i32<LX>(__float_as_int(v))); }
template <int LX>
TSFA_DEV double lane_xor_key(double v) { return lane_xor_f64<LX>(v); }

template <int E, int J, typename K>
TSFA_DEV void sortk_stage_regs(K (&key)[E], int g0, int k) {
#pragma unroll
    for (int e = 0; e < E; ++e) {
        if ((e & J) != 0) continue;
        const int f = e | J;
        const bool up = (((g0 + e) & k) == 0);
        const K lo = sort_min(key[e], key[f]), hi = sort_max(key[e], key[f]);
        key[e] = up ? lo : hi;
        key[f] = up ? hi : lo;
    }
}
template <int E, int LX, typename K>
TSFA_DEV void sortk_stage_lanes(K (&key)[E], int g0, int k, int j) {
    const bool lower = ((g0 & j) == 0);
#pragma unroll
    for (int e = 0; e < E; ++e) {
        const K o = lane_xor_key<LX>(key[e]);
        const bool up = (((g0 + e) & k) == 0);
        const K lo = sort_min(key[e], o), hi = sort_max(key[e], o);
        key[e] = (lower == up) ? lo : hi;
    }
}
template <int E, typename K>
TSFA_DEV void blk_sort_keys_regs(const Blk &b, K (&key)[E], K *xchg) {
    const int np2 = E * b.nt;
    const int g0 = b.tid * E;
    for (int k = 2; k <= np2; k <<= 1) {
        for (int j = k >> 1; j > 0; j >>= 1) {
            if (j < E) {
                switch (j) {
                case 1: if (E > 1) sortk_stage_regs<E, (E > 1 ? 1 : 0)>(key, g0, k); break;
                case 2: if (E > 2) sortk_stage_regs<E, (E > 2 ? 2 : 0)>(key, g0, k); break;
                case 4: if (E > 4) sortk_stage_regs<E, (E > 4 ? 4 : 0)>(key, g0, k); break;
                case 8: if (E > 8) sortk_stage_regs<E, (E > 8 ? 8 : 0)>(key, g0, k); break;
                default: break;
                }
            } else if (j < 64 * E) {
                switch (j / E) {
                case 1: sortk_stage_lanes<E, 1>(key, g0, k, j); break;
                case 2: sortk_stage_lanes<E, 2>(key, g0, k, j); break;
                case 4: sortk_stage_lanes<E, 4>(key, g0, k, j); break;
                case 8: sortk_stage_lanes<E, 8>(key, g0, k, j); break;
                case 16: sortk_stage_lanes<E, 16>(key, g0, k, j); break;
                default: sortk_stage_lanes<E, 32>(key, g0, k, j); break;
                }
            } else {
                blk_sync();
#pragma unroll
                for (int e = 0; e < E; ++e) xchg[g0 + e] = key[e];
                blk_sync();
                const bool lower = ((g0 & j) == 0);
#pragma unroll
                for (int e = 0; e < E; ++e) {
                    const K o = xchg[(g0 + e) ^ j];
                    const bool up = (((g0 + e) & k) == 0);
                    const K lo = sort_min(key[e], o), hi = sort_max(key[e], o);
                    key[e] = (lower == up) ? lo : hi;
                }
            }
        }
    }
}
template <int E, typename K>
TSFA_DEVN void blk_sorted_copy_regs_e(const Blk &b, const K *src, int n, K *dst) {
    K key[E];
#pragma unroll
    for (int e = 0; e < E; ++e) {
        const int g = b.tid * E + e;
        key[e] = (g < n) ? src[g] : (K)TSFA_INF;
    }
    blk_sort_keys_regs<E>(b, key, dst);
    blk_sync();
#pragma unroll
    for (int e = 0; e < E; ++e) dst[b.tid * E + e] = key[e];
    blk_sync();
}
template <typename K>
TSFA_DEV bool blk_sorted_copy_regs(const Blk &b, const K *src, int n, K *dst, int np2) {
    if (np2 == 2 * b.nt) { blk_sorted_copy_regs_e<2>(b, src, n, dst); return true; }
    if (np2 == 4 * b.nt) { blk_sorted_copy_regs_e<4>(b, src, n, dst); return true; }
    if (np2 == 8 * b.nt) { blk_sorted_copy_regs_e<8>(b, src, n, dst); return true; }
    if (np2 == 16 * b.nt) { blk_sorted_copy_regs_e<16>(b, src, n, dst); return true; }
    return false;
}
#endif

TSFA_DEV void tsfa_sincospi(double x, double *s, double *c) {
#if TSFA_GPU
    sincospi(x, s, c);
#else
    const double q = floor(x * 2.0 + 0.5);
    const double r = x - q * 0.5;
    const int qi = ((int)q) & 3;
    const double sr = sin(M_PI * r), cr = cos(M_PI * r);
    switch (qi) {
    case 0: *s = sr; *c = cr; break;
    case 1: *s = cr; *c = -sr; break;
    case 2: *s = -sr; *c = -cr; break;
    default: *s = -cr; *c = sr; break;
    }
#endif
}

TSFA_DEV double tsfa_lgamma(double x) {
    const double c[9] = {0.99999999999980993,  676.5203681218851,     -1259.1392167224028,
                         771.32342877765313,   -176.61502916214059,   12.507343278686905,
                         -0.13857109526572012, 9.9843695780195716e-6, 1.5056327351493116e-7};
    if (x < 0.5) return log(M_PI / fabs(sin(M_PI * x))) - tsfa_lgamma(1.0 - x);
    x -= 1.0;
    double a = c[0];
    const double t = x + 7.5;
    for (int i = 1; i < 9; ++i) a += c[i] / (x + (double)i);
    return 0.5 * log(2.0 * M_PI) + (x + 0.5) * log(t) - t + log(a);
}

TSFA_DEV double tsfa_betacf(double a, double b, double x) {
    const double FPMIN = 1e-300;
    const double qab = a + b, qap = a + 1.0, qam = a - 1.0;
    double c = 1.0, d = 1.0 - qab * x / qap;
    if (fabs(d) < FPMIN) d = FPMIN;
    d = 1.0 / d;
    double h = d;
    for (int m = 1; m <= 10000; ++m) {
        const double m2 = 2.0 * m;
        double aa = m * (b - m) * x / ((qam + m2) * (a + m2));
        d = 1.0 + aa * d;
        if (fabs(d) < FPMIN) d = FPMIN;
        c = 1.0 + aa / c;
        if (fabs(c) < FPMIN) c = FPMIN;
        d = 1.0 / d;
        h *= d * c;
        aa = -(a + m) * (qab + m) * x / ((a + m2) * (qap + m2));
        d = 1.0 + aa * d;
        if (fabs(d) < FPMIN) d = FPMIN;
        c = 1.0 + aa / c;
        if (fabs(c) < FPMIN) c = FPMIN;
        d = 1.0 / d;
        const double del = d * c;
        h *= del;
        if (fabs(del - 1.0) < 1e-16) break;
    }
    return h;
}

TSFA_DEV double tsfa_betainc(double a, double b, double x) {
    if (x != x) return TSFA_NAN;
    if (x <= 0.0) return 0.0;
    if (x >= 1.0) return 1.0;
    const double lbt = tsfa_lgamma(a + b) - tsfa_lgamma(a) - tsfa_lgamma(b) + a * log(x) + b * log1p(-x);
    if (x < (a + 1.0) / (a + b + 2.0)) return exp(lbt) * tsfa_betacf(a, b, x) / a;
    return 1.0 - exp(lbt) * tsfa_betacf(b, a, 1.0 - x) / b;
}

TSFA_DEV double tsfa_t_pvalue2(double t, double df) {
    if (t != t || !(df > 0.0)) return TSFA_NAN;
    if (isinf(t)) return 0.0;
    return tsfa_betainc(0.5 * df, 0.5, df / (df + t * t));
}
// ... 183 lines not shown
```

### tsfresh_amd/csrc/tsfa_kernels.hip

```cpp
#include <hip/hip_runtime.h>

#include "fam_ar.h"
#include "fam_ar_dd.h"
#include "fam_basic.h"
#include "fam_cwt.h"
#include "fam_entropy.h"
#include "fam_seq.h"
#include "fam_perm.h"
#include "fam_mprofile.h"
#include "fam_sort.h"
#include "fam_spectral.h"
#include "fam_general.h"
#include "tsfa_launch.h"
#include "tsfa_layout.h"

#include <algorithm>

#if defined(TSFA_LONG)
#define TSFA_GS_PARAMS , unsigned char *__restrict__ gsc, size_t gslot
#define TSFA_GS_ARGS , gsc, gslot
#define TSFA_SERIES_BEGIN                                                           \
    unsigned char *const tsfa_base = gsc + (size_t)blockIdx.x * gslot;             \
    for (int64_t wi_ = blockIdx.x; wi_ < n_series; wi_ += gridDim.x) {             \
        const int64_t sidx = sel ? (int64_t)sel[wi_] : wi_;
// ... 104 lines not shown
        blk_sync();
        const int64_t wn = wi + gridDim.x;
        if (wn < n_series) {
            sidx_n = sel ? (int64_t)sel[wn] : wn;
            const int64_t off = starts[sidx_n];
            n_n = (int)(ends[sidx_n] - off);
            if (prefetch) {
#pragma unroll
                for (int u = 0; u < 16; ++u) {
                    const int i = b.tid + u * b.nt;
                    pre[u] = (i < n_n) ? values[off + i] : (T)0;
                }
            }
        }
        fam_basic_series<5>(b, XsView<T>{xs}, n, specs, nspecs, out + sidx * ld, L.w, L.cum, L.altc, L.iw, dectab, hint_a, 0,
                            alt, L.stage, nullptr, 0, L.ctx, 0, 0);
        blk_sync();
    }
#endif
}

template <typename T>
__global__ void __launch_bounds__(512) __attribute__((amdgpu_waves_per_eu(4))) k_trend(const T *__restrict__ values, const int64_t *__restrict__ starts, const int64_t *__restrict__ ends, int64_t n_series, const int *__restrict__ sel,
                        const TsfaSpec *__restrict__ specs, int nspecs, double *__restrict__ out, int64_t ld, int maxn,
                        int hint_b, const double *__restrict__ times, const TsfaAltPlan alt, int n_loop, int skip_le TSFA_GS_PARAMS) {
    basic_body<T, 2>(values, starts, ends, n_series, sel, specs, nspecs, out, ld, nullptr, maxn, 0, hint_b, times, alt, n_loop, 0, 0, nullptr, skip_le TSFA_GS_ARGS);
}

#if !defined(TSFA_LONG)
template <typename T, int PART>
__device__ __forceinline__ void basic_rows_body(const T *__restrict__ values, const int64_t *__restrict__ starts, const int64_t *__restrict__ ends, int64_t n_series, const int *__restrict__ sel,
                        const TsfaSpec *__restrict__ specs, int nspecs, double *__restrict__ out, int64_t ld,
                        const double *__restrict__ dectab, int maxn, int hint_a, int hint_b,
                        const double *__restrict__ times, const TsfaAltPlan &alt, int n_loop, int n_count, int n_sum,
                        double *__restrict__ stats_out, int row_bytes) {
    const int row = (int)(threadIdx.x >> 4);
    const int64_t wi = (int64_t)blockIdx.x * (64 / TSFA_ROW_LANES) + row;
    if (wi >= n_series) return;
    const int64_t sidx = sel ? (int64_t)sel[wi] : wi;
    const int64_t off = starts[sidx];
    const int n = (int)(ends[sidx] - off);
    if (n > TSFA_ROW_MAXN) return;
    BasicRowLds L;
    L.carve(tsfa_smem + (size_t)row * (size_t)row_bytes, maxn, (int)sizeof(T), PART, (PART == 2) ? alt.small_w : 0);
    BlkRow b;
    b.tid = (int)(threadIdx.x & (TSFA_ROW_LANES - 1));
    b.nt = TSFA_ROW_LANES;
    b.red = L.red;
    b.np = nullptr;
    T *xs = (T *)L.xs;
    {
        const T *__restrict__ g = values + off;
        for (int i = b.tid; i < n; i += TSFA_ROW_LANES) xs[i] = g[i];
        blk_sync();
    }
    fam_basic_series<PART>(b, XsView<T>{xs}, n, specs, nspecs, out + sidx * ld, L.w, L.cum, L.altc, L.iw, dectab, hint_a,
                           hint_b, alt, (TsfaSpec *)nullptr, times ? times + off : nullptr, n_loop, L.ctx, n_count, n_sum,
                           stats_out ? stats_out + sidx * TSFA_STATS_N : nullptr);
}

#if !defined(TSFA_ROWS_WPE)
#define TSFA_ROWS_WPE 4
#endif
template <typename T>
__global__ void __launch_bounds__(64) __attribute__((amdgpu_waves_per_eu(TSFA_ROWS_WPE))) k_basic_rows(const T *__restrict__ values, const int64_t *__restrict__ starts, const int64_t *__restrict__ ends, int64_t n_series, const int *__restrict__ sel,
                        const TsfaSpec *__restrict__ specs, int nspecs, double *__restrict__ out, int64_t ld,
                        const double *__restrict__ dectab, int maxn, int hint_a, int n_loop, int n_count, int n_sum,
                        double *__restrict__ stats_out, int row_bytes) {
    TsfaAltPlan alt;
    alt.nkeys = 0; alt.want_p = 0; alt.nq = 0; alt.small_w = 0;
    basic_rows_body<T, 1>(values, starts, ends, n_series, sel, specs, nspecs, out, ld, dectab, maxn, hint_a, 0, nullptr, alt, n_loop,
                          n_count, n_sum, stats_out, row_bytes);
}

template <typename T>
__global__ void __launch_bounds__(64) __attribute__((amdgpu_waves_per_eu(TSFA_ROWS_WPE))) k_trend_rows(const T *__restrict__ values, const int64_t *__restrict__ starts, const int64_t *__restrict__ ends, int64_t n_series, const int *__restrict__ sel,
                        const TsfaSpec *__restrict__ specs, int nspecs, double *__restrict__ out, int64_t ld, int maxn,
                        int hint_b, const double *__restrict__ times, const TsfaAltPlan alt, int n_loop, int row_bytes) {
    basic_rows_body<T, 2>(values, starts, ends, n_series, sel, specs, nspecs, out, ld, nullptr, maxn, 0, hint_b, times, alt, n_loop, 0, 0,
                          nullptr, row_bytes);
}
#endif

template <typename T>
__global__ void __launch_bounds__(1024) k_sort(const T *__restrict__ values, const int64_t *__restrict__ starts, const int64_t *__restrict__ ends, int64_t n_series, const int *__restrict__ sel,
                       const TsfaSpec *__restrict__ specs, int nspecs, double *__restrict__ out, int64_t ld, int maxn,
                       const TsfaCqPlan cqplan, int n_loop, int w_doubles, double *__restrict__ pf_buf,
                       int *__restrict__ pf_count, int pf_slot, int pf_cap, const unsigned short *__restrict__ perm_buf, int perm_stride,
                       const double *__restrict__ stats_in, int pe_hint TSFA_GS_PARAMS) {
    TSFA_SERIES_BEGIN
    const int64_t off = starts[sidx];
    const int n = (int)(ends[sidx] - off);
    SortLds L;
    L.carve(tsfa_base, maxn, blockDim.x, (int)sizeof(T), w_doubles);
    TSFA_TICKS_BEGIN();
    Blk b{(int)threadIdx.x, (int)blockDim.x, L.red, L.np};
    T *xs = (T *)L.xs;
    {
        const T *__restrict__ g = values + off;
        for (int i = b.tid; i < n; i += b.nt) xs[i] = g[i];
        blk_sync();
    }
    fam_sort_series<T>(b, xs, n, specs, nspecs, out + sidx * ld, (T *)L.srt, L.w, L.iw, cqplan, L.cq, L.stage,
                       n_loop, L.ctx, w_doubles, FrDefer{pf_buf, pf_count, pf_slot, (long long)sidx, 0, pf_cap},
                       perm_buf ? perm_buf + (size_t)sidx * (size_t)perm_stride : nullptr,
                       stats_in ? stats_in + sidx * TSFA_STATS_N : nullptr, pe_hint);
    TSFA_TICKS_END();
    TSFA_SERIES_END
}

#if !defined(TSFA_LONG)
template <typename T>
__global__ void __launch_bounds__(1024) k_perm(const T *__restrict__ values, const int64_t *__restrict__ starts, const int64_t *__restrict__ ends, int64_t n_series, const int *__restrict__ sel,
                       const TsfaSpec *__restrict__ specs, int nspecs, double *__restrict__ out, int64_t ld, int maxn, int tau) {
    TSFA_SERIES_BEGIN
    const int64_t off = starts[sidx];
    const int n = (int)(ends[sidx] - off);
    PermLds L;
    L.carve(tsfa_base, maxn, blockDim.x, (int)sizeof(T), TSFA_PE_HIST_WORDS, TSFA_PE_LOGS + TSFA_PE_MAXD + 1);
    TSFA_TICKS_BEGIN();
    Blk b{(int)threadIdx.x, (int)blockDim.x, L.red, nullptr};
    T *xs = (T *)L.xs;
    {
        const T *__restrict__ g = values + off;
        for (int i = b.tid; i < n; i += b.nt) xs[i] = g[i];
        blk_sync();
    }
    fam_perm_series<T>(b, xs, n, specs, nspecs, out + sidx * ld, tau, L.iw, L.ltab);
    TSFA_TICKS_END();
    TSFA_SERIES_END
}
#endif

template <typename T>
__global__ void __launch_bounds__(256) k_mprofile(const T *__restrict__ values, const int64_t *__restrict__ starts, const int64_t *__restrict__ ends, int64_t n_series, const int *__restrict__ sel,
                           const TsfaSpec *__restrict__ specs, int nspecs, double *__restrict__ out, int64_t ld, int maxn TSFA_GS_PARAMS) {
    TSFA_SERIES_BEGIN
    const int64_t off = starts[sidx];
    const int n = (int)(ends[sidx] - off);
    MpLds L;
    L.carve(tsfa_base, maxn, (int)sizeof(T));
    TSFA_TICKS_BEGIN();
    Blk b{(int)threadIdx.x, (int)blockDim.x, L.red, L.np};
    T *xs = (T *)L.xs;
    {
        const T *__restrict__ g = values + off;
        for (int i = b.tid; i < n; i += b.nt) xs[i] = g[i];
        blk_sync();
    }
    fam_mprofile_series(b, XsView<T>{xs}, n, specs, nspecs, out + sidx * ld, L.w);
    TSFA_TICKS_END();
    TSFA_SERIES_END
}

template <typename T, bool BL>
__global__ void __launch_bounds__(1024) k_spectral(const T *__restrict__ values, const int64_t *__restrict__ starts, const int64_t *__restrict__ ends, int64_t n_series, const int *__restrict__ sel,
                           const TsfaSpec *__restrict__ specs, int nspecs, double *__restrict__ out, int64_t ld,
                           int maxn, int dft_n, double *__restrict__ gscratch, int gscratch_n, int bl_min,
                           const double *__restrict__ twc, const double *__restrict__ tws, int hint_a, int hint_b,
                           const double *__restrict__ consts TSFA_GS_PARAMS) {
    TSFA_SERIES_BEGIN
    const int64_t off = starts[sidx];
    const int n = (int)(ends[sidx] - off);
    SpectralLds L;
    L.carve(tsfa_base, maxn, dft_n, (int)sizeof(T));
    TSFA_TICKS_BEGIN();
    Blk b{(int)threadIdx.x, (int)blockDim.x, L.red, nullptr};
    T *xs = (T *)L.xs;
    {
        const T *__restrict__ g = values + off;
        for (int i = b.tid; i < n; i += b.nt) xs[i] = g[i];
        blk_sync();
    }
    double *gs = gscratch ? gscratch + (size_t)blockIdx.x * (size_t)gscratch_n : nullptr;
    fam_spectral_series<T, BL>(b, xs, n, specs, nspecs, out + sidx * ld, L.Xr, L.Xi, L.tc, L.ts, L.win, L.pxx, L.iw, twc, tws,
                        hint_a, hint_b, gs, consts ? consts + TSFA_CONSTS_HANN : nullptr, L.chirp_tab(), bl_min);
    TSFA_TICKS_END();
    TSFA_SERIES_END
}

template <typename T>
__global__ void __launch_bounds__(1024) k_ar(const T *__restrict__ values, const int64_t *__restrict__ starts, const int64_t *__restrict__ ends, int64_t n_series, const int *__restrict__ sel,
                     const TsfaSpec *__restrict__ specs, int nspecs, double *__restrict__ out, int64_t ld, int maxn,
                     int P, int hint_acf, int hint_pacf, int hint_adf, int n_loop, long long *__restrict__ deg_list,
                     int *__restrict__ deg_count, const double *__restrict__ stats_in TSFA_GS_PARAMS) {
    TSFA_SERIES_BEGIN
// ... 578 lines not shown
    __syncthreads();
    for (int i = threadIdx.x; i < TSFA_LEN_STATS; i += blockDim.x) {
        if (i == 1) atomicMin(&stats[1], acc[1]);
        else if (i >= 3 && i < 3 + TSFA_N_LEN_CLASSES) atomicAdd((unsigned long long *)&stats[i], (unsigned long long)acc[i]);
        else atomicMax(&stats[i], acc[i]);
    }
}

__global__ void __launch_bounds__(256) k_class_fill(const int64_t *__restrict__ starts, const int64_t *__restrict__ ends, int64_t n_series,
                                                    const TsfaClassMap g, int *__restrict__ cursor, int *__restrict__ sel) {
    for (int64_t s = (int64_t)blockIdx.x * blockDim.x + threadIdx.x; s < n_series;
         s += (int64_t)gridDim.x * blockDim.x) {
        const int grp = g.group_of[tsfa_len_class_dev(ends[s] - starts[s])];
        sel[g.base[grp] + atomicAdd(&cursor[grp], 1)] = (int)s;
    }
}

#endif

#define TSFA_LAUNCH_CHECK()                       \
    do {                                          \
        hipError_t e_ = hipGetLastError();        \
        if (e_ != hipSuccess) return (int)e_;     \
    } while (0)

template <typename K>
static int set_lds(K kern, size_t bytes) {
    if (bytes > 64 * 1024) {
        hipError_t e = hipFuncSetAttribute(reinterpret_cast<const void *>(kern),
                                           hipFuncAttributeMaxDynamicSharedMemorySize, (int)bytes);
        if (e != hipSuccess) return (int)e;
    }
    return 0;
}

#if defined(TSFA_LONG)
#define TSFA_KLAUNCH(kern, lds, ...)                                                                       \
    do {                                                                                                   \
        const size_t slot_ = ((size_t)(lds) + 255) & ~(size_t)255;                                          \
        const int64_t slots_ = (int64_t)(a.long_bytes / slot_);                                            \
        if (!a.long_scratch || slots_ < 1) return -2;                                                      \
        const dim3 lgrid_((unsigned)std::min<int64_t>(a.n_series, std::min<int64_t>(slots_, 2048)));       \
        kern<<<lgrid_, nt, 0, st>>>(__VA_ARGS__, a.long_scratch, slot_);                                   \
    } while (0)
#else
#define TSFA_KLAUNCH(kern, lds, ...)                           \
    do {                                                       \
        if ((rc = set_lds(kern, lds))) return rc;              \
        kern<<<grid, nt, lds, st>>>(__VA_ARGS__);              \
    } while (0)
#endif

template <typename T>
static int launch_all_t(const TsfaLaunch &a, const T *values) {
    hipStream_t st = (hipStream_t)a.stream;
    const dim3 grid((unsigned)a.n_series);
    const int nt = a.nt;
    int rc = 0;
    (void)grid; (void)rc;
    if (a.fam == TSFA_FAM_BASIC) {
        BasicLds L;
        const size_t lds = L.carve(nullptr, a.maxn, nt, (int)sizeof(T), 1);
        if (a.hint_c == 0 && nt <= 256) {
#if defined(TSFA_LONG)
            TSFA_KLAUNCH(k_basic_lite<T>, lds, values, a.starts, a.ends, a.n_series, a.sel, a.specs, a.nspecs, a.out, a.ld,
                         a.dectab, a.maxn, a.hint_a);
#else
            if ((rc = set_lds(k_basic_lite<T>, lds))) return rc;
            const int64_t resident = std::max<int64_t>(1, std::min<int64_t>(32, (int64_t)(TSFA_LDS_LIMIT / std::max<size_t>(lds, 1))));
            const dim3 pgrid((unsigned)std::min<int64_t>(a.n_series, 256 * resident));
            k_basic_lite<T><<<pgrid, nt, lds, st>>>(values, a.starts, a.ends, a.n_series, a.sel, a.specs, a.nspecs, a.out, a.ld,
                                                     a.dectab, a.maxn, a.hint_a);
#endif
        } else {
            TSFA_KLAUNCH(k_basic<T>, lds, values, a.starts, a.ends, a.n_series, a.sel, a.specs, a.nspecs, a.out, a.ld, a.dectab,
                         a.maxn, a.hint_a, a.hint_c, a.hint_d, a.hint_e, a.stats_out, a.skip_le);
        }
    } else if (a.fam == TSFA_FAM_TREND) {
        BasicLds L;
        const size_t lds = L.carve(nullptr, a.maxn, nt, (int)sizeof(T), 2, a.alt.small_w);
        TSFA_KLAUNCH(k_trend<T>, lds, values, a.starts, a.ends, a.n_series, a.sel, a.specs, a.nspecs, a.out, a.ld, a.maxn,
                     a.hint_b, a.times, a.alt, a.hint_c, a.skip_le);
    } else if (a.fam == TSFA_FAM_SORT) {
        SortLds L;
        const int wd = (a.hint_a >= 320) ? a.hint_a : 1280;
        const size_t lds = L.carve(nullptr, a.maxn, nt, (int)sizeof(T), wd);
        TSFA_KLAUNCH(k_sort<T>, lds, values, a.starts, a.ends, a.n_series, a.sel, a.specs, a.nspecs, a.out, a.ld, a.maxn, a.cq,
                     a.hint_c, wd, a.pf_buf, a.pf_count, a.pf_slot, a.pf_cap, a.perm_buf, a.perm_stride, a.stats_in, a.hint_d);
    } else if (a.fam == TSFA_FAM_SPECTRAL) {
        SpectralLds L;
        const size_t lds = L.carve(nullptr, a.maxn, a.dft_n, (int)sizeof(T));
        if (a.gscratch != nullptr) {
            auto kfn = k_spectral<T, true>;
#if defined(TSFA_LONG)
            TSFA_KLAUNCH(kfn, lds, values, a.starts, a.ends, a.n_series, a.sel, a.specs, a.nspecs, a.out, a.ld, a.maxn,
                         a.dft_n, a.gscratch, a.gscratch_n, a.bluestein_min, a.twc, a.tws, a.hint_a, a.hint_b, a.consts);
#else
            if ((rc = set_lds(kfn, lds))) return rc;
            const int64_t slots = std::max<int64_t>(a.gscratch_slots, 1);
            for (int64_t c0 = 0; c0 < a.n_series; c0 += slots) {
                const int64_t nc = std::min<int64_t>(slots, a.n_series - c0);
                const int64_t s0 = a.sel ? 0 : c0;
                kfn<<<dim3((unsigned)nc), nt, lds, st>>>(values, a.starts + s0, a.ends + s0, nc, a.sel ? a.sel + c0 : nullptr, a.specs,
                                                        a.nspecs, a.out + s0 * a.ld, a.ld, a.maxn, a.dft_n, a.gscratch,
                                                        a.gscratch_n, a.bluestein_min, a.twc, a.tws, a.hint_a, a.hint_b, a.consts);
            }
#endif
        } else {
            auto kfn = k_spectral<T, false>;
            TSFA_KLAUNCH(kfn, lds, values, a.starts, a.ends, a.n_series, a.sel, a.specs, a.nspecs, a.out, a.ld, a.maxn,
                         a.dft_n, a.gscratch, a.gscratch_n, a.bluestein_min, a.twc, a.tws, a.hint_a, a.hint_b, a.consts);
        }
    } else if (a.fam == TSFA_FAM_AR) {
        ArLds L;
        const size_t lds = L.carve(nullptr, a.maxn, a.ar_P, (int)sizeof(T), nt);
        TSFA_KLAUNCH(k_ar<T>, lds, values, a.starts, a.ends, a.n_series, a.sel, a.specs, a.nspecs, a.out, a.ld, a.maxn, a.ar_P,
                     a.hint_a, a.hint_b, a.hint_c, a.hint_d, a.deg_list, a.deg_count, a.stats_in);
    } else if (a.fam == TSFA_FAM_ENTROPY) {
#if defined(TSFA_LONG)
        if (a.ent_cnt == 4) {
            EntropyHugeSlot H;
            const size_t slot_ = (H.carve(nullptr, a.maxn) + 255) & ~(size_t)255;
            const int64_t slots_ = (int64_t)(a.long_bytes / slot_);
            if (!a.long_scratch || slots_ < 1) return -2;
            const size_t hl = entropy_huge_lds_bytes(a.maxn);
            auto kfn = kl_entropy_hbits<T>;
            hipError_t e = hipFuncSetAttribute(reinterpret_cast<const void *>(kfn), hipFuncAttributeMaxDynamicSharedMemorySize, (int)hl);
            if (e != hipSuccess) return (int)e;
            const dim3 hgrid((unsigned)std::min<int64_t>(a.n_series, std::min<int64_t>(slots_, 512)));
            kfn<<<hgrid, 1024, hl, st>>>(values, a.starts, a.ends, a.n_series, a.sel, a.specs, a.nspecs, a.out, a.ld, a.maxn, a.stats_in,
                                         a.long_scratch, slot_);
            TSFA_LAUNCH_CHECK();
            return 0;
        }
#endif
        EntropyLds L;
#if defined(TSFA_LONG)
        const size_t lds = L.carve(nullptr, a.maxn, a.ent_cnt, 4);
#else
        const size_t lds = L.carve(nullptr, a.maxn, a.ent_cnt);
#endif
#if !defined(TSFA_LONG)
        if (a.ent_cnt == 3) {
            auto kfn = k_entropy_bits<T, TSFA_ENTB_QW_LONG>;
            TSFA_KLAUNCH(kfn, lds, values, a.starts, a.ends, a.n_series, a.sel, a.specs, a.nspecs, a.out, a.ld, a.maxn,
                         (unsigned short *)nullptr, 0, a.stats_in);
        } else if (a.ent_cnt == 2) {
            auto kfn = k_entropy_bits<T, TSFA_ENTB_QW>;
            TSFA_KLAUNCH(kfn, lds, values, a.starts, a.ends, a.n_series, a.sel, a.specs, a.nspecs, a.out, a.ld, a.maxn,
                         a.perm_buf, a.perm_stride, a.stats_in);
        } else
#endif
        if (a.ent_fast) {
            auto kfn = k_entropy<T, true>;
            TSFA_KLAUNCH(kfn, lds, values, a.starts, a.ends, a.n_series, a.sel, a.specs, a.nspecs, a.out, a.ld, a.maxn, a.ent_cnt, a.stats_in);
        } else {
            auto kfn = k_entropy<T, false>;
            TSFA_KLAUNCH(kfn, lds, values, a.starts, a.ends, a.n_series, a.sel, a.specs, a.nspecs, a.out, a.ld, a.maxn, a.ent_cnt, a.stats_in);
        }
    } else if (a.fam == TSFA_FAM_SEQ) {
        SeqLds L;
        const size_t lds = L.carve(nullptr, a.seq.grows ? 0 : 1, a.seq.stride, a.seq.ttotal, a.seq.etotal, (nt + 63) >> 6);
#if !defined(TSFA_LONG)
        if (a.seq.grows) {
            if (!a.seq_rows) return -2;
            auto kfn = k_seq<T, true>;
            TSFA_KLAUNCH(kfn, lds, values, a.starts, a.ends, a.n_series, a.sel, a.out, a.ld, a.seq, a.stats_in, a.seq_rows);
        } else
#endif
        {
            auto kfn = k_seq<T, false>;
// ... 75 lines not shown
    __shared__ double red[TSFA_RED_DOUBLES];
    __shared__ NpScratch nps;
    Blk b{(int)threadIdx.x, (int)blockDim.x, red, &nps};
    GenSlot S;
    S.carve(scratch + (size_t)blockIdx.x * slot_doubles, maxn, g);
    for (int64_t sidx = blockIdx.x; sidx < n_series; sidx += gridDim.x) {
        const int64_t off = starts[sidx];
        const int n = (int)(ends[sidx] - off);
        const T *gv = values + off;
        fam_general_series(b, [=](int i) { return (double)gv[i]; }, n, specs, nspecs, out + sidx * ld, S, g, pool);
        __syncthreads();
    }
}

size_t tsfa_general_slot_doubles(int maxn, const TsfaGenPlan &g) {
    GenSlot S;
    return S.carve(nullptr, maxn, g);
}

int tsfa_launch_general(const TsfaLaunch &a, const TsfaGenPlan &g, double *scratch, size_t slot_doubles, int slots, const double *pool) {
    hipStream_t st = (hipStream_t)a.stream;
    const unsigned grid = (unsigned)std::max<int64_t>(1, std::min<int64_t>(a.n_series, slots));
    if (a.dtype == 0)
        k_general<float><<<grid, 64, 0, st>>>((const float *)a.values, a.starts, a.ends, a.n_series, a.specs, a.nspecs, a.out, a.ld, a.maxn, g,
                                              scratch, slot_doubles, pool);
    else
        k_general<double><<<grid, 64, 0, st>>>((const double *)a.values, a.starts, a.ends, a.n_series, a.specs, a.nspecs, a.out, a.ld, a.maxn, g,
                                               scratch, slot_doubles, pool);
    TSFA_LAUNCH_CHECK();
    return 0;
}
#else
template <typename T>
static int launch_ar_degenerate_t(const TsfaLaunch &a, const T *values) {
    hipStream_t st = (hipStream_t)a.stream;
    int rc;
    ArDdLds D;
    const int P = a.ar_P_dd > 0 ? a.ar_P_dd : a.ar_P;
    size_t dlds = D.carve(nullptr, P);
    unsigned dgrid = (unsigned)std::min<int64_t>(a.n_series, 4096);
    if (a.dd_scratch != nullptr) {
        dlds = (size_t)TSFA_RED_DOUBLES * sizeof(double) + 64;
        dgrid = (unsigned)std::max<int64_t>(1, std::min<int64_t>(a.n_series, a.dd_slots));
    }
    if ((rc = set_lds(k_ar_degenerate<T>, dlds))) return rc;
    k_ar_degenerate<T><<<dgrid, 64, dlds, st>>>(values, a.starts, a.ends, a.specs, a.nspecs, a.out, a.ld, P, a.deg_list,
                                                a.deg_count, (a.hint_c >> 1) & 3, a.dd_scratch);
    TSFA_LAUNCH_CHECK();
    return 0;
}
int tsfa_launch_ar_degenerate(const TsfaLaunch &a) {
    if (!(a.hint_c || a.ar_has_coef)) return 0;
    if (a.dtype == 0) return launch_ar_degenerate_t<float>(a, (const float *)a.values);
    return launch_ar_degenerate_t<double>(a, (const double *)a.values);
}

int tsfa_launch_langevin_dd(const TsfaLaunch &a) {
    if (!a.pf_buf) return 0;
    hipStream_t st = (hipStream_t)a.stream;
    const unsigned grid = (unsigned)std::min<int64_t>((a.n_series + 63) / 64, 4096);
    k_langevin_dd<<<grid, 64, 0, st>>>(a.pf_buf, a.pf_count, a.pf_slot, a.pf_cap, a.specs, a.nspecs, a.out, a.ld);
    TSFA_LAUNCH_CHECK();
    return 0;
}

size_t tsfa_entropy_lds_bytes(int maxn, int with_cnt) {
    if (with_cnt == 5) {
        EntropyLds L;
        return L.carve(nullptr, maxn, 0, 4);
    }
    if (with_cnt == 4) {
        EntropyHugeSlot H;
        return H.carve(nullptr, maxn);
    }
    EntropyLds L;
    return L.carve(nullptr, maxn, with_cnt);
}

size_t tsfa_seq_lds_bytes(const TsfaSeqGroup &g) {
    SeqLds L;
    return L.carve(nullptr, g.grows ? 0 : 1, g.stride, g.ttotal, g.etotal);
}

size_t tsfa_family_lds_bytes(int fam, int maxn, int nt, int aux) {
    switch (fam) {
    case TSFA_FAM_BASIC: { BasicLds L; return L.carve(nullptr, maxn, nt, 8, 1); }
    case TSFA_FAM_TREND: { BasicLds L; return L.carve(nullptr, maxn, nt, 8, 2, aux); }
    case TSFA_FAM_SORT: { SortLds L; return L.carve(nullptr, maxn, nt); }
    case TSFA_FAM_SPECTRAL: { SpectralLds L; return L.carve(nullptr, maxn, aux); }
    case TSFA_FAM_AR: { ArLds L; return L.carve(nullptr, maxn, aux, 8, nt); }
    case TSFA_FAM_CWT: {
        CwtPeaksLayout L;
        const size_t lds16 = L.carve(nullptr, maxn, aux, 8, 2);
        return lds16 > TSFA_LDS_LIMIT ? L.carve(nullptr, maxn, aux, 8, 4) : lds16;
    }
    case TSFA_FAM_MPROFILE: { MpLds L; return L.carve(nullptr, maxn, aux); }
    default: return 0;
    }
}

int tsfa_launch_family(const TsfaLaunch &a) {
    if (a.dtype == 0) return launch_all_t<float>(a, (const float *)a.values);
    return launch_all_t<double>(a, (const double *)a.values);
}

template <typename T>
static int launch_order_stats_t(const TsfaLaunch &a, const T *values) {
    hipStream_t st = (hipStream_t)a.stream;
    const dim3 grid((unsigned)((a.n_series + 3) / 4));
    if (a.maxn <= 256)
        k_order_stats<T, 4><<<grid, 256, 0, st>>>(values, a.starts, a.ends, a.n_series, a.sel, a.specs, a.nspecs, a.out, a.ld);
    else if (a.maxn <= 1024)
        k_order_stats<T, 16><<<grid, 256, 0, st>>>(values, a.starts, a.ends, a.n_series, a.sel, a.specs, a.nspecs, a.out, a.ld);
    else if (a.maxn <= 2048)
        k_order_stats<T, 32><<<grid, 256, 0, st>>>(values, a.starts, a.ends, a.n_series, a.sel, a.specs, a.nspecs, a.out, a.ld);
    else
        return -1;
    TSFA_LAUNCH_CHECK();
    return 0;
}
template <typename T>
static int launch_stream_t(const TsfaLaunch &a, const T *values) {
    hipStream_t st = (hipStream_t)a.stream;
    const dim3 grid((unsigned)((a.n_series + 3) / 4));
    const int wm = a.nspecs > 0 ? 1 : 0;
#define TSFA_STREAM_CASE(EE) k_stream<T, EE><<<grid, 256, 0, st>>>(values, a.starts, a.ends, a.n_series, a.sel, a.bspecs, a.nbspecs, a.specs, a.nspecs, wm, a.out, a.ld)
    if (a.maxn <= 256) TSFA_STREAM_CASE(4);
    else if (a.maxn <= 512) TSFA_STREAM_CASE(8);
    else if (a.maxn <= 1024) TSFA_STREAM_CASE(16);
    else if (a.maxn <= 2048) TSFA_STREAM_CASE(32);
    else return -1;
#undef TSFA_STREAM_CASE
    TSFA_LAUNCH_CHECK();
    return 0;
}
int tsfa_launch_stream(const TsfaLaunch &a) {
    if (a.dtype == 0) return launch_stream_t<float>(a, (const float *)a.values);
    return launch_stream_t<double>(a, (const double *)a.values);
}
int tsfa_stream_calc_ok(int calc) {
    switch (calc) {
    case TSFA_C_SUM_VALUES: case TSFA_C_MEAN: case TSFA_C_LENGTH: case TSFA_C_STANDARD_DEVIATION: case TSFA_C_VARIANCE:
    case TSFA_C_ROOT_MEAN_SQUARE: case TSFA_C_MAXIMUM: case TSFA_C_ABSOLUTE_MAXIMUM: case TSFA_C_MINIMUM:
    case TSFA_C_ABS_ENERGY: case TSFA_C_VARIATION_COEFFICIENT: case TSFA_C_QUERY_SIMILARITY_COUNT: case TSFA_C_MEDIAN:
        return 1;
    default: return 0;
    }
}

size_t tsfa_perm_lds_bytes(int maxn, int nt, int elem_bytes) {
    PermLds L;
    return L.carve(nullptr, maxn, nt, elem_bytes, TSFA_PE_HIST_WORDS, TSFA_PE_LOGS + TSFA_PE_MAXD + 1);
}
template <typename T>
static int launch_perm_t(const TsfaLaunch &a, const T *values) {
    hipStream_t st = (hipStream_t)a.stream;
    const dim3 grid((unsigned)a.n_series);
    const int nt = a.nt;
    const size_t lds = tsfa_perm_lds_bytes(a.maxn, nt, (int)sizeof(T));
    int rc = 0;
    if ((rc = set_lds(k_perm<T>, lds))) return rc;
    k_perm<T><<<grid, nt, lds, st>>>(values, a.starts, a.ends, a.n_series, a.sel, a.specs, a.nspecs, a.out, a.ld, a.maxn, a.hint_d >> 8);
    TSFA_LAUNCH_CHECK();
    return 0;
}
int tsfa_launch_perm(const TsfaLaunch &a) {
// ... 78 lines not shown
```

### tsfresh_amd/csrc/tsfa_launch.h

```cpp
#ifndef TSFA_LAUNCH_H
#define TSFA_LAUNCH_H

#include <stddef.h>
#include <stdint.h>

#include "tsfa_specs.h"
#include "fam_seq.h"

#define TSFA_N_LEN_CLASSES 11
#define TSFA_LEN_STATS (3 + 3 * TSFA_N_LEN_CLASSES)
static inline int tsfa_len_class(long long l) {
    int c = 0;
    while (c < TSFA_N_LEN_CLASSES - 1 && l > (64LL << c)) ++c;
    return c;
}
struct TsfaClassMap {
    int group_of[TSFA_N_LEN_CLASSES];
    int base[TSFA_N_LEN_CLASSES];
};

struct TsfaLaunch {
    int fam;
    int dtype;
    const void *values;
    const int64_t *starts;
    const int64_t *ends;
    int64_t n_series;
    const int *sel;
    const TsfaSpec *specs;
    int nspecs;
    const TsfaSpec *bspecs;
    int nbspecs;
    double *out;
    int64_t ld;
    int maxn;
    int skip_le;
    int nt;
    void *stream;
    const double *dectab;
    TsfaCqPlan cq;
    TsfaAltPlan alt;
    const double *times;
    const double *twc, *tws;
    int dft_n;
    double *gscratch;
    int gscratch_n;
    TsfaSeqGroup seq;
    unsigned char *seq_rows;
    int ar_P;
    int ar_P_dd;
    double *dd_scratch;
    int dd_slots;
    int ar_has_coef;
    long long *deg_list;
    int *deg_count;
    double *stats_out;
    const double *stats_in;
    const double *consts;
    double *pf_buf;
    int *pf_count;
    int pf_slot;
    int pf_cap;
    unsigned short *perm_buf;
    int perm_stride;
    int64_t gscratch_slots;
    int bluestein_min;
    int cwt_rowv;
    int hint_a, hint_b, hint_c, hint_d, hint_e;
    unsigned char *long_scratch;
    size_t long_bytes;
    int ent_cnt;
    int ent_fast;
};

struct TsfaCwtLaunch {
    int dtype;
    const void *values;
    const int64_t *starts, *ends;
    int64_t n_series;
    const double *W;
    int S4, C;
    const int *cols;
    const int *coeff_idx;
    double *out;
    int64_t ld;
    void *stream;
};

size_t tsfa_family_lds_bytes(int fam, int maxn, int nt, int aux);
size_t tsfa_entropy_lds_bytes(int maxn, int with_cnt);
size_t tsfa_seq_lds_bytes(const TsfaSeqGroup &g);
int tsfa_launch_family(const TsfaLaunch &a);
int tsfa_launch_rows(const TsfaLaunch &a);
int tsfa_launch_family_long(const TsfaLaunch &a);
size_t tsfa_general_slot_doubles(int maxn, const TsfaGenPlan &g);
int tsfa_launch_general(const TsfaLaunch &a, const TsfaGenPlan &g, double *scratch, size_t slot_doubles, int slots, const double *pool);
int tsfa_launch_ar_degenerate(const TsfaLaunch &a);
int tsfa_launch_langevin_dd(const TsfaLaunch &a);
int tsfa_launch_perm(const TsfaLaunch &a);
size_t tsfa_perm_lds_bytes(int maxn, int nt, int elem_bytes);
int tsfa_launch_stream(const TsfaLaunch &a);
int tsfa_stream_calc_ok(int calc);
int tsfa_launch_order_stats(const TsfaLaunch &a);
int tsfa_launch_cwt(const TsfaCwtLaunch &a);
int tsfa_launch_fill_nan(double *out, int64_t n_rows, int64_t n_cols, int64_t ld, void *stream, double value,
                         const int *cols, int n_fill);
int tsfa_launch_len_stats(const int64_t *starts, const int64_t *ends, int64_t n_series, long long *stats, void *stream);
int tsfa_launch_class_fill(const int64_t *starts, const int64_t *ends, int64_t n_series, const TsfaClassMap &g, int *cursor,
                           int *sel, void *stream);

#endif
```

### tsfresh_amd/csrc/tsfa_layout.h

```cpp
#ifndef TSFA_LAYOUT_H
#define TSFA_LAYOUT_H

#include <stddef.h>
#include <stdint.h>

#include "tsfa_common.h"
#include "fam_cwt.h"
#include "fam_seq.h"
#include "fam_mprofile.h"
#include "tsfa_entb_params.h"

#if defined(__HIPCC__)
#define TSFA_HD __host__ __device__ inline
#else
#define TSFA_HD inline
#endif

#define TSFA_LDS_LIMIT (160 * 1024)

struct LdsCarve {
    unsigned char *base;
    size_t off;
    template <class U>
    TSFA_HD U *take(size_t count) {
        off = (off + 15) & ~(size_t)15;
        U *r = (U *)(base + off);
        off += count * sizeof(U);
        return r;
    }
};

TSFA_HD int tsfa_pow2_ceil(int n) {
    int p = 1;
    while (p < n) p <<= 1;
    return p;
}

struct BasicLds {
    double *red; NpScratch *np; void *xs; double *w; double *cum; double *altc; int *iw; TsfaSpec *stage; double *ctx;
    TSFA_HD size_t carve(unsigned char *base, int maxn, int nt, int xs_bytes = 8, int part = 3, int small_w = 0) {
        LdsCarve c{base, 0};
        red = c.take<double>(nt <= 64 ? 2 : TSFA_RED_DOUBLES);
        xs = c.take<unsigned char>((size_t)maxn * xs_bytes);
        size_t wb = (part & 2) ? (size_t)maxn * sizeof(double) : (size_t)maxn * xs_bytes;
        if ((part & 2) && small_w) wb = (size_t)(nt + 2 * 16 + 8) * sizeof(double);
        if (wb < sizeof(NpScratch)) wb = sizeof(NpScratch);
        unsigned char *u = c.take<unsigned char>(wb);
        w = (double *)u;
        cum = w;
        np = (NpScratch *)u;
        altc = (part & 2) ? c.take<double>(8 * 16) : nullptr;
        ctx = c.take<double>(32);
        iw = c.take<int>((4 * nt > 256) ? 4 * nt : 256);
#if defined(TSFA_SPEC_LDS)
        stage = c.take<TsfaSpec>(TSFA_SPEC_BATCH);
#else
        stage = nullptr;
#endif
        return c.off;
    }
};

#define TSFA_ROW_BINS 64
struct BasicRowLds {
    double *red; void *xs; double *w; double *cum; double *altc; int *iw; double *ctx;
    TSFA_HD static size_t row_bytes(int maxn, int xs_bytes, int part, int small_w) {
        BasicRowLds L;
        const size_t used = L.carve(nullptr, maxn, xs_bytes, part, small_w);
        return ((used + 127) & ~(size_t)127) + 64;
    }
    TSFA_HD size_t carve(unsigned char *base, int maxn, int xs_bytes, int part, int small_w) {
        LdsCarve c{base, 0};
        red = c.take<double>(2);
        xs = c.take<unsigned char>((size_t)maxn * xs_bytes);
        size_t wb = (part & 2) ? (size_t)maxn * sizeof(double) : (size_t)maxn * xs_bytes;
        if ((part & 2) && small_w) wb = (size_t)(TSFA_ROW_LANES + 2 * 16 + 8) * sizeof(double);
        if (wb < 64) wb = 64;
        w = (double *)c.take<unsigned char>(wb);
        cum = w;
        altc = (part & 2) ? c.take<double>(8 * 16) : nullptr;
        ctx = c.take<double>(32);
        iw = c.take<int>((part & 2) ? 16 * 6 * 2 : TSFA_ROW_BINS);
        return c.off;
    }
};

struct SortLds {
    double *red; NpScratch *np; void *xs; void *srt; double *w; int *iw; double *cq; TsfaSpec *stage; double *ctx;
    TSFA_HD size_t carve(unsigned char *base, int maxn, int nt, int xs_bytes = 8, int w_doubles = 1280) {
        (void)nt;
        LdsCarve c{base, 0};
        red = c.take<double>(TSFA_RED_DOUBLES);
        np = c.take<NpScratch>(1);
        xs = c.take<unsigned char>((size_t)maxn * xs_bytes);
        srt = c.take<unsigned char>((size_t)tsfa_pow2_ceil(maxn) * xs_bytes);
        w = c.take<double>(w_doubles);
        iw = (int *)w;
        cq = c.take<double>(5 * TSFA_CQ_MAX);
        ctx = c.take<double>(8);
#if defined(TSFA_SPEC_LDS)
        stage = c.take<TsfaSpec>(TSFA_SPEC_BATCH);
#else
        stage = nullptr;
#endif
        return c.off;
    }
};

struct SpectralLds {
    double *red; void *xs; double *Xr; double *Xi; double *tc; double *ts; double *win; double *pxx; int *iw;
    TSFA_HD size_t carve(unsigned char *base, int maxn, int dft_n, int xs_bytes = 8) {
        LdsCarve c{base, 0};
        red = c.take<double>(TSFA_RED_DOUBLES);
        xs = c.take<unsigned char>((size_t)maxn * xs_bytes);
        const int nx = (maxn / 2 + 2 > 260) ? maxn / 2 + 2 : 260;
        Xr = c.take<double>(nx);
        Xi = c.take<double>(nx);
        const int nd = (dft_n > 256) ? dft_n : (dft_n > 0 ? 256 : 2);
        tc = c.take<double>(nd);
        ts = c.take<double>(nd);
        win = c.take<double>(256);
        pxx = c.take<double>(dft_n > 0 ? 260 : 132);
        iw = (int *)(void *)win;
        has_chirp_tab = (nd == 256 && dft_n > 0);
        return c.off;
    }
    bool has_chirp_tab = false;
    TSFA_HD double *chirp_tab() const { return has_chirp_tab ? tc : nullptr; }
};

struct ArLds {
    double *red; NpScratch *np; double *xc; double *aw; double *part; int part_doubles;
    TSFA_HD static int scratch_doubles(int P) { return (P * (P - 1)) / 2 + 8 * P + 64 + 8 + 48 + 32; }
    TSFA_HD size_t carve(unsigned char *base, int maxn, int P, int xs_bytes = 8, int nt = 64) {
        LdsCarve c{base, 0};
        red = c.take<double>(TSFA_RED_DOUBLES);
        xc = (double *)(void *)c.take<unsigned char>((size_t)(maxn + 64 + 16) * xs_bytes);
        const size_t ab = (size_t)scratch_doubles(P) * sizeof(double);
        unsigned char *u = c.take<unsigned char>(ab > sizeof(NpScratch) ? ab : sizeof(NpScratch));
        aw = (double *)u;
        np = (NpScratch *)u;
        part_doubles = (nt > 64) ? 72 * ((nt + 63) / 64) : 0;
        part = part_doubles ? c.take<double>((size_t)part_doubles) : nullptr;
        return c.off;
    }
};

struct ArDdLds {
    double *red; double *scratch;
    TSFA_HD static int scratch_doubles(int P) { return 4 * P * P + 19 * (P + 1) + P + 10; }
    TSFA_HD size_t carve(unsigned char *base, int P) {
        LdsCarve c{base, 0};
        red = c.take<double>(TSFA_RED_DOUBLES);
        scratch = c.take<double>((size_t)scratch_doubles(P));
        return c.off;
    }
};

struct EntropyLds {
    double *red; NpScratch *np; double *xs; double *thr; unsigned short *perm; unsigned int *refs; unsigned int *cnt;
    TSFA_HD size_t carve(unsigned char *base, int maxn, int with_cnt, int idx_bytes = 2) {
        LdsCarve c{base, 0};
        red = c.take<double>(TSFA_RED_DOUBLES);
        thr = c.take<double>(56);
        xs = c.take<double>(maxn + 4);
        const int np2 = tsfa_pow2_ceil(maxn);
        const int nperm = ((np2 > 64) ? np2 : 64) + 32;
        perm = (unsigned short *)(void *)c.take<unsigned char>((size_t)nperm * (size_t)idx_bytes);
        if (with_cnt == 2 || with_cnt == 3) {
            refs = nullptr;
            const size_t cb = (with_cnt == 2 ? entb_work_words(maxn)
                                             : entb_work_words(maxn, TSFA_ENTB_QW_LONG + 1, entb_kround(maxn, TSFA_ENTB_MAXK, TSFA_ENTB_MAXWAVES))) * sizeof(unsigned int);
            unsigned char *u = c.take<unsigned char>(cb > sizeof(NpScratch) ? cb : sizeof(NpScratch));
            np = (NpScratch *)u;
            cnt = (unsigned int *)u;
        } else if (with_cnt) {
            refs = c.take<unsigned int>(nperm);
            const size_t cb = (size_t)(maxn + 16) * ((maxn <= 1024) ? 4 : 3) * sizeof(unsigned int);
            unsigned char *u = c.take<unsigned char>(cb > sizeof(NpScratch) ? cb : sizeof(NpScratch));
// ... 99 lines not shown
```

Baseline: 2.808 million series/sec.

## Run sort family as single-wavefront blocks with slim LDS and 16-bit order view

Changes the sort family's default block size from 128 to 64 threads and adds templated single-wave modes. In these modes block barriers become LDS waitcnts, the reduction and NpScratch LDS regions are shrunk or aliased onto the work buffer, and, when a precomputed permutation is available, a 16-bit index view replaces the sorted copy. The goal is to cut LDS footprint and barrier overhead so more blocks fit per CU. In exchange each series gets fewer threads, and aliasing NpScratch with the work buffer risks corruption if both are live at the same time.

```diff
diff --git a/__graft_entry__.py b/__graft_entry__.py
--- a/__graft_entry__.py
+++ b/__graft_entry__.py
@@ -23,6 +23,8 @@
     emul_roll_lib.load()
     import emul_mprofile_lib
     emul_mprofile_lib.load()
+    import emul_sort_lib
+    emul_sort_lib.load()
     import tsfresh_amd
     from tsfresh_amd import _native
     lib = _native.load()
diff --git a/tsfresh_amd/csrc/fam_ar.h b/tsfresh_amd/csrc/fam_ar.h
--- a/tsfresh_amd/csrc/fam_ar.h
+++ b/tsfresh_amd/csrc/fam_ar.h
@@ -13,16 +13,6 @@
 TSFA_DEV int ar_tri(int i, int j) { return ((i * (i + 1)) >> 1) + j; }
 TSFA_DEV int ar_tri_doubles(int P) { return (P * (P - 1)) / 2; }
 
-TSFA_DEV void ar_sync(const Blk &b) {
-#if TSFA_GPU && !defined(TSFA_LONG)
-    if (b.nt <= 64) {
-        asm volatile("s_waitcnt lgkmcnt(0)" ::: "memory");
-        return;
-    }
-#endif
-    (void)b;
-    blk_sync();
-}
 
 TSFA_DEV bool chol_factor(double *G, int p) {
     for (int j = 0; j < p; ++j) {
diff --git a/tsfresh_amd/csrc/fam_sort.h b/tsfresh_amd/csrc/fam_sort.h
--- a/tsfresh_amd/csrc/fam_sort.h
+++ b/tsfresh_amd/csrc/fam_sort.h
@@ -260,7 +260,7 @@
     double *sy = sx + r;
     double *cnt = sy + r;
     double *lows = cnt + r + 1;
-    blk_sync();
+    ar_sync(b);
     for (int j = b.tid; j <= r; j += b.nt) {
         const double q = np_linspace_at(0.0, 1.0, r + 1, j);
         edges[j] = pd_quantile_sorted(srt1, ns, q);
@@ -268,7 +268,7 @@
     long long *isx = (long long *)(void *)sx, *isy = (long long *)(void *)sy, *icnt = (long long *)(void *)cnt,
               *isxl = (long long *)(void *)lows, *isyl = isxl + r;
     for (int j = b.tid; j < r; j += b.nt) { isx[j] = 0; isy[j] = 0; icnt[j] = 0; isxl[j] = 0; isyl[j] = 0; }
-    blk_sync();
+    ar_sync(b);
     double bad = 0.0;
     for (int j = b.tid; j < r; j += b.nt) bad += (edges[j] < edges[j + 1]) ? 0.0 : 1.0;
     bad = blk_sum(b, bad);
@@ -303,13 +303,13 @@
             isx[bin] += xh; isy[bin] += yh; isxl[bin] += xl; isyl[bin] += yl; icnt[bin] += 1;
 #endif
         }
-        blk_sync();
+        ar_sync(b);
         for (int j = b.tid; j < r; j += b.nt) {
             const double vx = fx_value(isx[j], isxl[j], fx), vy = fx_value(isy[j], isyl[j], fy);
             const double vc = (double)icnt[j];
             sx[j] = vx; sy[j] = vy; cnt[j] = vc;
         }
-        blk_sync();
+        ar_sync(b);
     }
     return true;
 }
@@ -330,7 +330,7 @@
     double *tmp = cc + (m + 1);
     if (!friedrich_bin_means(b, xs, n, srt1, r, fw)) return;
     if (b.tid == 0) flag[0] = 0.0;
-    blk_sync();
+    ar_sync(b);
     const int rmax = (df.slot_doubles - TSFA_PF_HDR) / 2;
 #if TSFA_GPU
     if (b.tid < 64) {
@@ -476,10 +476,10 @@
         }
     }
 #endif
-    blk_sync();
+    ar_sync(b);
     if (flag[0] != 0.0)
         for (int c = 0; c <= m; ++c) coef[c] = cc[c];
-    blk_sync();
+    ar_sync(b);
 }
 
 #define TSFA_CQ_REFINE 9.5367431640625e-07
@@ -529,7 +529,7 @@
             if (e < plan.n) cq[5 * e] = v; else cq[5 * (e - plan.n) + 1] = v;
         }
     }
-    blk_sync();
+    ar_sync(b);
     double s = (n > 1) ? (xs[n - 1] - xs[0]) / (double)(n - 1) : 0.0;
     if (!(fabs(s) <= 1.7976931348623157e308)) s = 0.0;
     const double sa = fabs(s);
@@ -601,7 +601,7 @@
                 a[5 * jj + 4] = (jj == j && ((refine >> jj) & 16)) ? w2 : a[5 * jj + 4];
             }
         }
-        blk_sync();
+        ar_sync(b);
         if (b.tid == 0) {
 #pragma unroll
             for (int j = 0; j < 4; ++j) {
@@ -622,7 +622,7 @@
             }
         }
     }
-    blk_sync();
+    ar_sync(b);
 }
 
 enum { TSFA_SCTX_SYM = 0, TSFA_SCTX_NUNIQUE, TSFA_SCTX_MULTI_VALS, TSFA_SCTX_MULTI_PTS, TSFA_SCTX_SUM_VALS, TSFA_SCTX_SUM_PTS,
@@ -662,22 +662,46 @@
 }
 
 template <class ST>
+struct OrdView {
+    const ST *p;
+    const unsigned short *o;
+    TSFA_MEM double operator[](int i) const { return (double)p[o[i]]; }
+};
+template <class ST, bool ORD> struct SortedView { typedef XsView<ST> type; };
+template <class ST> struct SortedView<ST, true> { typedef OrdView<ST> type; };
+
+template <class ST, bool ORD = false>
 TSFA_DEV void fam_sort_series(const Blk &b, const ST *xs_raw, int n, const TsfaSpec *specs, int nspecs,
                               double *out_row, ST *srt_raw, double *w, int *iw, const TsfaCqPlan &cqplan, double *cq,
                               TsfaSpec *stage, int n_loop = -1, double *ctx = nullptr, int w_doubles = 1280,
                               FrDefer df = FrDefer{nullptr, nullptr, TSFA_PF_HDR + 2 * TSFA_FRIEDRICH_MAX_R, 0, 0},
                               const unsigned short *perm_in = nullptr, const double *stats = nullptr, int pe_hint = 0) {
-    const int hist_words = 2 * w_doubles;
+    const bool own_np = (b.np != nullptr) && ((const void *)b.np != (const void *)w);
+    const int hist_words = own_np ? 2 * w_doubles : 2 * (w_doubles - 64);
     const int nloop = (n_loop >= 0 && ctx != nullptr) ? n_loop : nspecs;
+    typedef typename SortedView<ST, ORD>::type SV;
     const XsView<ST> xs{xs_raw};
-    const XsView<ST> srt{srt_raw};
+    unsigned short *ord = (unsigned short *)(void *)srt_raw;
+    (void)ord;
+    SV srt;
+    if constexpr (ORD) { srt.p = xs_raw; srt.o = ord; } else { srt.p = srt_raw; }
     const int np2 = next_pow2(n);
     TSFA_TICKER(tk, 0);
-    blk_sync();
+    ar_sync(b);
     auto build_sorted_copy = [&]() {
+        if constexpr (ORD) {
+            if (n >= 3) {
+                for (int i = b.tid; i < n; i += b.nt) ord[i] = perm_in[i];
+            } else if (b.tid == 0) {
+                const bool swap = (n == 2) && (xs_raw[1] < xs_raw[0]);
+                ord[0] = swap ? 1 : 0;
+                if (n == 2) ord[1] = swap ? 0 : 1;
+            }
+            ar_sync(b);
+        } else
         if (perm_in != nullptr && n >= 3) {
             for (int i = b.tid; i < np2; i += b.nt) srt_raw[i] = (i < n) ? xs_raw[perm_in[i]] : (ST)TSFA_INF;
-            blk_sync();
+            ar_sync(b);
         } else
 #if TSFA_GPU
         if (!blk_sorted_copy_regs(b, xs_raw, n, srt_raw, np2))
@@ -828,17 +852,17 @@
         } break;
         case TSFA_C_PERMUTATION_ENTROPY: {
             const int tau = (int)p0, D = (int)p1;
-            if (pe_hint != 0) { TSFA_TICK(tk, b, sp.calc); continue; }
+            if (ORD || pe_hint != 0) { TSFA_TICK(tk, b, sp.calc); continue; }
             const int num = (n >= D) ? ((n - D) / tau + 1) : 0;
             if (num <= 0) { v = TSFA_NAN; break; }
             int fact = 1;
             for (int k = 2; k <= D; ++k) fact *= k;
             const bool wide = num > 65535;
             const int per_pass = wide ? hist_words : 2 * hist_words;
-            if (fact > 16 * per_pass && sizeof(ST) >= sizeof(int)) {
+            if (!ORD && fact > 16 * per_pass && sizeof(ST) >= sizeof(int)) {
                 int *codes_s = (int *)(void *)srt_raw;
                 const int cp2 = next_pow2(num);
-                blk_sync();
+                ar_sync(b);
                 for (int t = b.tid; t < cp2; t += b.nt) codes_s[t] = (t < num) ? perm_code(xs_raw + t * tau, D, fact) : 0x7FFFFFFF;
                 blk_bitonic_sort(b, codes_s, cp2);
                 double es = 0.0;
@@ -851,7 +875,7 @@
                     es += pr * log(pr);
                 }
                 v = -blk_sum(b, es);
-                blk_sync();
+                ar_sync(b);
                 build_sorted_copy();
                 break;
             }
@@ -867,17 +891,17 @@
             }
             TSFA_TICK(tp, b, 236);
             const int LT = 64;
-            double *ltab = b.np->leaf_sum;
-            blk_sync();
+            double *ltab = own_np ? b.np->leaf_sum : w + (w_doubles - 64);
+            ar_sync(b);
             for (int c = b.tid; c < LT; c += b.nt) ltab[c] = (c > 0) ? log((double)c / (double)num) : 0.0;
-            blk_sync();
+            ar_sync(b);
             TSFA_TICK(tp, b, 237);
             double e = 0.0;
             for (int base = 0; base < fact; base += per_pass) {
                 const int top = (fact - base < per_pass) ? (fact - base) : per_pass;
-                blk_sync();
+                ar_sync(b);
                 for (int k = b.tid; k < (wide ? top : (top + 1) >> 1); k += b.nt) iw[k] = 0;
-                blk_sync();
+                ar_sync(b);
                 if (in_regs) {
 #pragma unroll
                     for (int u = 0; u < 8; ++u) {
@@ -902,7 +926,7 @@
                         }
                     }
                 }
-                blk_sync();
+                ar_sync(b);
                 if (fact <= num) {
                     for (int k = b.tid; k < top; k += b.nt) {
                         const unsigned wv = (unsigned)iw[wide ? k : (k >> 1)];
@@ -957,7 +981,7 @@
                     }
                     pos = lo;
                 }
-                const XsView<ST> sr = srt;
+                const SV sr = srt;
                 df.spec = s;
                 friedrich_coeffs(b, xs, n, [=](int i) { return sr[i < pos ? i : i + 1]; }, m, r, w, fr_coef, df);
                 fr_valid = true;
@@ -974,7 +998,7 @@
         TSFA_TICK(tk, b, sp.calc);
     }
     if (nloop < nspecs) {
-        blk_sync();
+        ar_sync(b);
         sort_epilogue(b, specs, nloop, nspecs, n, srt, ctx, cq, out_row);
     }
 }
diff --git a/tsfresh_amd/csrc/tsfa_api.cpp b/tsfresh_amd/csrc/tsfa_api.cpp
--- a/tsfresh_amd/csrc/tsfa_api.cpp
+++ b/tsfresh_amd/csrc/tsfa_api.cpp
@@ -68,6 +68,7 @@
     bool length_classes = true;
     bool stats_share = true;
     bool perm_share = true;
+    int sort_waves = 1;
     bool select = true;
     bool bluestein = true;
     bool cwt_mfma = false;
@@ -391,6 +392,7 @@
     else if (n == "row_form") o.row_form = on;
     else if (n == "seq_rows") o.seq_rows = (value < 0.0) ? -1 : (on ? 1 : 0);
     else if (n == "entropy_route") { if (value != 0.0 && value != 1.0 && value != 2.0) return fail(TSFA_ERR_INVALID, "entropy_route: 0, 1 or 2"); o.entropy_route = (int)value; }
+    else if (n == "sort_waves") { if (value != 1.0 && value != 2.0) return fail(TSFA_ERR_INVALID, "sort_waves: 1 or 2"); o.sort_waves = (int)value; }
     else if (n == "bluestein_min") o.bluestein_min = value > 0.0 ? (int)std::min(value, 32767.0) : 0;
     else if (n == "gscratch_slots") o.gscratch_slots = value > 0.0 ? (int)std::min(value, 2147483647.0) : 0;
     else if (n == "host_chunks") o.host_chunks = value > 0.0 ? (int)std::min(value, (double)TSFA_MAX_CHUNKS) : 0;
@@ -618,9 +620,10 @@
                 a.nt = (maxn > 4096) ? nt_8k[f] : nt_4k[f];
             }
             if (maxn <= 2048) {
-                static const int pref[TSFA_N_FAMILIES] = {64, 128, 128, 64, 256, 256, 128, 64, 256};
+                static const int pref[TSFA_N_FAMILIES] = {64, 64, 128, 64, 256, 256, 128, 64, 256};
                 const int cap = std::max(64, ((maxn / 4 + 63) / 64) * 64);
                 a.nt = std::min(pref[f], cap);
+                if (f == TSFA_FAM_SORT && plan->opt.sort_waves == 2) a.nt = std::min(128, cap);
             }
             if (TSFA_LAB_ONLY(plan->opt.nt[f] >= 64)) a.nt = plan->opt.nt[f];
             a.stream = fst;
@@ -839,6 +842,11 @@
                     }
                 }
             }
+            if (f == TSFA_FAM_SORT && !use_long) {
+                a.sort_mode = (maxn <= 2048 && a.nt == 64 && plan->opt.sort_waves == 1 && !TSFA_LAB_ONLY(plan->opt.nt[f] >= 64))
+                                  ? ((a.perm_buf != nullptr && a.hint_d != 0) ? 2 : 1) : 0;
+                lds = tsfa_sort_lds_bytes(a, dtype == TSFA_F32 ? 4 : 8);
+            }
             if (!(plan->stream_ok && (f == TSFA_FAM_SORT || f == TSFA_FAM_BASIC) && maxn <= 2048 && g <= TSFA_N_LEN_CLASSES && stream_done[g])) {
                 tsfa_launch_info li;
                 li.family = f;
@@ -852,7 +860,7 @@
                              : (f == TSFA_FAM_CWT) ? a.cwt_rowv
                              : (f == TSFA_FAM_SEQ) ? (seq_group | (seq_grows << 8))
                              : (f == TSFA_FAM_SPECTRAL) ? (a.gscratch != nullptr ? 1 : 0)
-                             : (f == TSFA_FAM_SORT) ? (a.hint_d != 0 ? 1 : 0)
+                             : (f == TSFA_FAM_SORT) ? ((a.hint_d != 0 ? 1 : 0) | (a.sort_mode << 1))
                              : (f == TSFA_FAM_AR) ? (a.dd_scratch != nullptr ? 1 : 0) : 0;
                 plan->launches.push_back(li);
             }
diff --git a/tsfresh_amd/csrc/tsfa_common.h b/tsfresh_amd/csrc/tsfa_common.h
--- a/tsfresh_amd/csrc/tsfa_common.h
+++ b/tsfresh_amd/csrc/tsfa_common.h
@@ -113,6 +113,17 @@
     asm volatile("s_waitcnt vmcnt(0) lgkmcnt(0)" ::: "memory");
     __syncthreads();
 #endif
+}
+
+TSFA_DEV void ar_sync(const Blk &b) {
+#if TSFA_GPU && !defined(TSFA_LONG)
+    if (b.nt <= 64) {
+        asm volatile("s_waitcnt lgkmcnt(0)" ::: "memory");
+        return;
+    }
+#endif
+    (void)b;
+    blk_sync();
 }
 
 #if TSFA_GPU
@@ -753,7 +764,7 @@
 TSFA_DEV void blk_bitonic_sort(const Blk &b, K *a, int npow2) {
     for (int k = 2; k <= npow2; k <<= 1) {
         for (int j = k >> 1; j > 0; j >>= 1) {
-            blk_sync();
+            ar_sync(b);
             for (int t = b.tid; t < (npow2 >> 1); t += b.nt) {
                 const int i = ((t & ~(j - 1)) << 1) | (t & (j - 1));
                 const int l = i | j;
@@ -766,7 +777,7 @@
             }
         }
     }
-    blk_sync();
+    ar_sync(b);
 }
 
 template <class IDX>
@@ -1029,10 +1040,10 @@
                 default: sortk_stage_lanes<E, 32>(key, g0, k, j); break;
                 }
             } else {
-                blk_sync();
+                ar_sync(b);
 #pragma unroll
                 for (int e = 0; e < E; ++e) xchg[g0 + e] = key[e];
-                blk_sync();
+                ar_sync(b);
                 const bool lower = ((g0 & j) == 0);
 #pragma unroll
                 for (int e = 0; e < E; ++e) {
@@ -1054,10 +1065,10 @@
         key[e] = (g < n) ? src[g] : (K)TSFA_INF;
     }
     blk_sort_keys_regs<E>(b, key, dst);
-    blk_sync();
+    ar_sync(b);
 #pragma unroll
     for (int e = 0; e < E; ++e) dst[b.tid * E + e] = key[e];
-    blk_sync();
+    ar_sync(b);
 }
 template <typename K>
 TSFA_DEV bool blk_sorted_copy_regs(const Blk &b, const K *src, int n, K *dst, int np2) {
diff --git a/tsfresh_amd/csrc/tsfa_kernels.hip b/tsfresh_amd/csrc/tsfa_kernels.hip
--- a/tsfresh_amd/csrc/tsfa_kernels.hip
+++ b/tsfresh_amd/csrc/tsfa_kernels.hip
@@ -210,7 +210,7 @@
 }
 #endif
 
-template <typename T>
+template <typename T, int MODE>
 __global__ void __launch_bounds__(1024) k_sort(const T *__restrict__ values, const int64_t *__restrict__ starts, const int64_t *__restrict__ ends, int64_t n_series, const int *__restrict__ sel,
                        const TsfaSpec *__restrict__ specs, int nspecs, double *__restrict__ out, int64_t ld, int maxn,
                        const TsfaCqPlan cqplan, int n_loop, int w_doubles, double *__restrict__ pf_buf,
@@ -219,17 +219,18 @@
     TSFA_SERIES_BEGIN
     const int64_t off = starts[sidx];
     const int n = (int)(ends[sidx] - off);
+    const int nt = (MODE != 0) ? 64 : (int)blockDim.x;
     SortLds L;
-    L.carve(tsfa_base, maxn, blockDim.x, (int)sizeof(T), w_doubles);
+    L.carve(tsfa_base, maxn, nt, (int)sizeof(T), w_doubles, MODE == 2 ? 1 : 0, stats_in == nullptr ? 1 : 0);
     TSFA_TICKS_BEGIN();
-    Blk b{(int)threadIdx.x, (int)blockDim.x, L.red, L.np};
+    Blk b{(int)threadIdx.x, nt, L.red, L.np};
     T *xs = (T *)L.xs;
     {
         const T *__restrict__ g = values + off;
         for (int i = b.tid; i < n; i += b.nt) xs[i] = g[i];
-        blk_sync();
-    }
-    fam_sort_series<T>(b, xs, n, specs, nspecs, out + sidx * ld, (T *)L.srt, L.w, L.iw, cqplan, L.cq, L.stage,
+        ar_sync(b);
+    }
+    fam_sort_series<T, MODE == 2>(b, xs, n, specs, nspecs, out + sidx * ld, (T *)L.srt, L.w, L.iw, cqplan, L.cq, L.stage,
                        n_loop, L.ctx, w_doubles, FrDefer{pf_buf, pf_count, pf_slot, (long long)sidx, 0, pf_cap},
                        perm_buf ? perm_buf + (size_t)sidx * (size_t)perm_stride : nullptr,
                        stats_in ? stats_in + sidx * TSFA_STATS_N : nullptr, pe_hint);
@@ -974,11 +975,24 @@
         TSFA_KLAUNCH(k_trend<T>, lds, values, a.starts, a.ends, a.n_series, a.sel, a.specs, a.nspecs, a.out, a.ld, a.maxn,
                      a.hint_b, a.times, a.alt, a.hint_c, a.skip_le);
     } else if (a.fam == TSFA_FAM_SORT) {
-        SortLds L;
         const int wd = (a.hint_a >= 320) ? a.hint_a : 1280;
-        const size_t lds = L.carve(nullptr, a.maxn, nt, (int)sizeof(T), wd);
-        TSFA_KLAUNCH(k_sort<T>, lds, values, a.starts, a.ends, a.n_series, a.sel, a.specs, a.nspecs, a.out, a.ld, a.maxn, a.cq,
-                     a.hint_c, wd, a.pf_buf, a.pf_count, a.pf_slot, a.pf_cap, a.perm_buf, a.perm_stride, a.stats_in, a.hint_d);
+        const size_t lds = tsfa_sort_lds_bytes(a, (int)sizeof(T));
+#if !defined(TSFA_LONG)
+        if (a.sort_mode == 2) {
+            auto kfn = k_sort<T, 2>;
+            TSFA_KLAUNCH(kfn, lds, values, a.starts, a.ends, a.n_series, a.sel, a.specs, a.nspecs, a.out, a.ld, a.maxn, a.cq,
+                         a.hint_c, wd, a.pf_buf, a.pf_count, a.pf_slot, a.pf_cap, a.perm_buf, a.perm_stride, a.stats_in, a.hint_d);
+        } else if (a.sort_mode == 1) {
+            auto kfn = k_sort<T, 1>;
+            TSFA_KLAUNCH(kfn, lds, values, a.starts, a.ends, a.n_series, a.sel, a.specs, a.nspecs, a.out, a.ld, a.maxn, a.cq,
+                         a.hint_c, wd, a.pf_buf, a.pf_count, a.pf_slot, a.pf_cap, a.perm_buf, a.perm_stride, a.stats_in, a.hint_d);
+        } else
+#endif
+        {
+            auto kfn = k_sort<T, 0>;
+            TSFA_KLAUNCH(kfn, lds, values, a.starts, a.ends, a.n_series, a.sel, a.specs, a.nspecs, a.out, a.ld, a.maxn, a.cq,
+                         a.hint_c, wd, a.pf_buf, a.pf_count, a.pf_slot, a.pf_cap, a.perm_buf, a.perm_stride, a.stats_in, a.hint_d);
+        }
     } else if (a.fam == TSFA_FAM_SPECTRAL) {
         SpectralLds L;
         const size_t lds = L.carve(nullptr, a.maxn, a.dft_n, (int)sizeof(T));
@@ -1220,6 +1234,12 @@
     return L.carve(nullptr, g.grows ? 0 : 1, g.stride, g.ttotal, g.etotal);
 }
 
+size_t tsfa_sort_lds_bytes(const TsfaLaunch &a, int xs_bytes) {
+    SortLds L;
+    return L.carve(nullptr, a.maxn, a.nt, xs_bytes, (a.hint_a >= 320) ? a.hint_a : 1280, a.sort_mode == 2 ? 1 : 0,
+                   a.stats_in == nullptr ? 1 : 0);
+}
+
 size_t tsfa_family_lds_bytes(int fam, int maxn, int nt, int aux) {
     switch (fam) {
     case TSFA_FAM_BASIC: { BasicLds L; return L.carve(nullptr, maxn, nt, 8, 1); }
diff --git a/tsfresh_amd/csrc/tsfa_launch.h b/tsfresh_amd/csrc/tsfa_launch.h
--- a/tsfresh_amd/csrc/tsfa_launch.h
+++ b/tsfresh_amd/csrc/tsfa_launch.h
@@ -71,6 +71,7 @@
     size_t long_bytes;
     int ent_cnt;
     int ent_fast;
+    int sort_mode;
 };
 
 struct TsfaCwtLaunch {
@@ -90,6 +91,7 @@
 size_t tsfa_family_lds_bytes(int fam, int maxn, int nt, int aux);
 size_t tsfa_entropy_lds_bytes(int maxn, int with_cnt);
 size_t tsfa_seq_lds_bytes(const TsfaSeqGroup &g);
+size_t tsfa_sort_lds_bytes(const TsfaLaunch &a, int xs_bytes);
 int tsfa_launch_family(const TsfaLaunch &a);
 int tsfa_launch_rows(const TsfaLaunch &a);
 int tsfa_launch_family_long(const TsfaLaunch &a);
diff --git a/tsfresh_amd/csrc/tsfa_layout.h b/tsfresh_amd/csrc/tsfa_layout.h
--- a/tsfresh_amd/csrc/tsfa_layout.h
+++ b/tsfresh_amd/csrc/tsfa_layout.h
@@ -87,14 +87,24 @@
 
 struct SortLds {
     double *red; NpScratch *np; void *xs; void *srt; double *w; int *iw; double *cq; TsfaSpec *stage; double *ctx;
-    TSFA_HD size_t carve(unsigned char *base, int maxn, int nt, int xs_bytes = 8, int w_doubles = 1280) {
-        (void)nt;
-        LdsCarve c{base, 0};
-        red = c.take<double>(TSFA_RED_DOUBLES);
-        np = c.take<NpScratch>(1);
-        xs = c.take<unsigned char>((size_t)maxn * xs_bytes);
-        srt = c.take<unsigned char>((size_t)tsfa_pow2_ceil(maxn) * xs_bytes);
-        w = c.take<double>(w_doubles);
+    TSFA_HD size_t carve(unsigned char *base, int maxn, int nt, int xs_bytes = 8, int w_doubles = 1280, int ord16 = 0,
+                         int with_np = 1) {
+        LdsCarve c{base, 0};
+        const bool one_wave = nt <= 64;
+        red = c.take<double>(one_wave ? 2 : TSFA_RED_DOUBLES);
+        np = one_wave ? nullptr : c.take<NpScratch>(1);
+        xs = c.take<unsigned char>((size_t)maxn * xs_bytes);
+        srt = (one_wave && ord16) ? c.take<unsigned char>((size_t)maxn * sizeof(unsigned short))
+                                  : c.take<unsigned char>((size_t)tsfa_pow2_ceil(maxn) * xs_bytes);
+        if (one_wave) {
+            size_t wb = (size_t)w_doubles * sizeof(double);
+            if (with_np && wb < sizeof(NpScratch)) wb = sizeof(NpScratch);
+            unsigned char *u = c.take<unsigned char>(wb);
+            w = (double *)u;
+            np = with_np ? (NpScratch *)u : nullptr;
+        } else {
+            w = c.take<double>(w_doubles);
+        }
         iw = (int *)w;
         cq = c.take<double>(5 * TSFA_CQ_MAX);
         ctx = c.take<double>(8);
```

Result: faster. 2.957 million series/sec (median of 6 runs) (+5.3%).
